# TomBeacock/volumetric-renderer

Hardware: AMD Instinct MI355X
Metric: Gsamples/sec + fps, 512³ NRRD @ 1080p; achieved HBM GB/s vs peak (higher is better)
Workload: dtype f32

## Files before the change

include/vr/vr.h:

```cpp
#ifndef VR_VR_H
#define VR_VR_H

#include <stddef.h>
#include <stdint.h>

#ifdef __cplusplus
extern "C" {
#endif

#define VR_ABI_VERSION 9

#define VR_OK 0
#define VR_EINVAL (-22)
#define VR_ENOMEM (-12)
#define VR_ENODEV (-19)
#define VR_ENODATA (-61)
#define VR_EIO (-5)

enum vr_dtype {
    VR_DTYPE_I8 = 1,
    VR_DTYPE_U8 = 2,
    VR_DTYPE_I16 = 3,
    VR_DTYPE_U16 = 4,
    VR_DTYPE_I32 = 5,
// ... 32 lines not shown
    int32_t wave_shape;
    int32_t frames_in_flight;
    int32_t exact_gradient;
    int32_t depth_zero_to_one;
} vr_params;

typedef struct vr_stats {
    uint64_t rays;
    uint64_t samples;
    uint64_t shaded_samples;
    uint64_t steps;
    uint64_t skipped_samples;
} vr_stats;

int vr_abi_version(void);
void vr_params_default(vr_params *p);

typedef struct vr_ctx vr_ctx;
vr_ctx *vr_create(int device, uint32_t width, uint32_t height);
vr_ctx *vr_create_mask(uint32_t device_mask, uint32_t width, uint32_t height);
void vr_destroy(vr_ctx *ctx);
const char *vr_last_error(const vr_ctx *ctx);

int vr_resize(vr_ctx *ctx, uint32_t width, uint32_t height);
int vr_get_size(const vr_ctx *ctx, uint32_t *width, uint32_t *height);
int vr_get_device(const vr_ctx *ctx, int *device);
int vr_get_device_mask(const vr_ctx *ctx, uint32_t *device_mask);


int vr_set_volume(vr_ctx *ctx, const void *data, int dtype, uint32_t nx, uint32_t ny,
                  uint32_t nz, float vmin, float vmax);
int vr_set_volume_device(vr_ctx *ctx, const void *data_dev, int dtype, uint32_t nx,
                         uint32_t ny, uint32_t nz, float vmin, float vmax, void *stream);
int vr_generate_volume(vr_ctx *ctx, int kind, int dtype, uint32_t nx, uint32_t ny,
                       uint32_t nz, uint32_t seed, float *vmin_out, float *vmax_out);
uint64_t vr_volume_bytes(const vr_ctx *ctx);
int vr_debug_read_volume(vr_ctx *ctx, float *out_host);
int vr_debug_read_volume_native(vr_ctx *ctx, void *out_host);
int vr_debug_volume_info(const vr_ctx *ctx, uint32_t dims[3], float minmax[2], int *storage);

int vr_set_transfer_function(vr_ctx *ctx, const uint32_t *rgba8_srgb, uint32_t n);

int vr_set_slicing(vr_ctx *ctx, const float min_slice[3], const float max_slice[3]);


int vr_render(vr_ctx *ctx, const vr_camera *cam, const vr_params *p, void *out,
              int out_format);

int vr_render_device(vr_ctx *ctx, const vr_camera *cam, const vr_params *p, void *out_dev,
                     int out_format, uint32_t row_block, uint32_t rank, uint32_t nranks,
                     void *stream);
uint32_t vr_shard_rows(uint32_t height, uint32_t row_block, uint32_t nranks);
int vr_set_row_share(vr_ctx *ctx, uint32_t first_weight, uint32_t other_weight);
int vr_get_row_share(const vr_ctx *ctx, uint32_t *first_weight, uint32_t *other_weight);
uint32_t vr_shard_rows_ctx(const vr_ctx *ctx, uint32_t height, uint32_t row_block, uint32_t nranks);
int vr_assemble_rows(vr_ctx *ctx, const void *gathered_dev, void *out_dev, int out_format,
                     uint32_t row_block, uint32_t nranks, void *stream);

typedef struct vr_external_memory vr_external_memory;
int vr_import_memory_fd(vr_ctx *ctx, int fd, uint64_t size, uint64_t offset,
                        vr_external_memory **mem, void **dev_ptr);
int vr_release_external_memory(vr_ctx *ctx, vr_external_memory *mem);

typedef struct vr_memory_info {
    uint64_t volume_bytes;
    uint64_t field_bytes;
    uint64_t oblique_copy_bytes;
    uint64_t plain_copy_bytes;
    uint64_t stencil_copy_bytes;
    uint64_t skip_bytes;
    uint64_t derived_bytes;
    uint64_t budget_bytes;
    uint64_t builds;
    uint64_t evictions;
    uint64_t downgrades;
    uint64_t last_downgrade;
} vr_memory_info;
enum vr_derived {
    VR_DERIVED_FIELD = 1,
    VR_DERIVED_OBLIQUE_COPY = 2,
    VR_DERIVED_PLAIN_COPY = 3,
    VR_DERIVED_STENCIL_COPY = 4,
    VR_DERIVED_SKIP = 5,
    VR_DERIVED_YMAJOR_COPY = 6
};
#define VR_MEMORY_BUDGET_UNLIMITED (~(uint64_t)0)
#define VR_MEMORY_BUDGET_DEFAULT (~(uint64_t)0 - 1)
int vr_set_memory_budget(vr_ctx *ctx, uint64_t bytes);
int vr_memory_report(const vr_ctx *ctx, vr_memory_info *out);
int vr_prepare(vr_ctx *ctx, const vr_camera *cam, const vr_params *p);

int vr_count_work(vr_ctx *ctx, const vr_camera *cam, const vr_params *p, uint32_t row_block,
                  uint32_t rank, uint32_t nranks, vr_stats *out);

int vr_timing_enable(vr_ctx *ctx, int enable);
int vr_timing_read(vr_ctx *ctx, double *total_ms, uint64_t *launches);
int vr_timing_reset(vr_ctx *ctx);

const char *vr_kernel_name(const vr_ctx *ctx, const vr_params *p);

#ifdef __cplusplus
}
#endif

#endif
```

include/vr/vr_debug.h:

```cpp
#ifndef VR_VR_DEBUG_H
#define VR_VR_DEBUG_H

#include "vr.h"
#include "vr_dist.h"

#ifdef __cplusplus
extern "C" {
#endif

enum vr_knob {
    VR_KNOB_PIPELINE = 1,
    VR_KNOB_PAIR = 2,
    VR_KNOB_PAIR_LANES = 3,
    VR_KNOB_GRAD_FIELD = 4,
    VR_KNOB_U8_LAYOUT = 6,
    VR_KNOB_TILE_ORDER = 7,
    VR_KNOB_NARROW = 8,
    VR_KNOB_ALT_GEOMETRY = 9,
    VR_KNOB_MIP_INFLIGHT = 10
};

typedef struct vr_member_timing {
    int32_t device;
    uint64_t frames;
    double kernel_ms, render_ms, gather_ms, assemble_ms;
} vr_member_timing;
int vr_debug_timing_member(vr_ctx *ctx, int member, vr_member_timing *out);

enum vr_exchange { VR_EXCHANGE_RCCL = 0, VR_EXCHANGE_COPY = 1 };
vr_ctx *vr_debug_create_members(const int *devices, int n, uint32_t width, uint32_t height,
                                int exchange);
int vr_debug_fail_member(vr_ctx *ctx, int member, uint64_t frame);

int vr_debug_host_profile_enable(vr_ctx *ctx, int enable);
int vr_debug_host_profile_member(vr_ctx *ctx, int member, vr_dist_host_profile *out);

int vr_debug_set_knob(vr_ctx *ctx, int knob, int value);
int vr_debug_get_knob(const vr_ctx *ctx, int knob, int *value);

typedef struct vr_variant_facts {
    int32_t layout, mode;
    int32_t shade, count, skip, field, field_half, pipeline;
    int32_t tf_n, pair, mip_inflight;
} vr_variant_facts;
int vr_debug_variant_name(const vr_variant_facts *facts, char *buf, size_t n);
const char *vr_debug_last_kernel_name(const vr_ctx *ctx);

uint64_t vr_debug_ymajor_copy_bytes(const vr_ctx *ctx);

#ifdef __cplusplus
}
#endif

#endif
```

volumetric-renderer_amd/csrc/vr_api.hip:

```cpp
#include "../../include/vr/vr.h"
#include "../../include/vr/vr_debug.h"
#include "../../include/vr/vr_modes.h"
#include "../../include/vr/vr_iso.h"
#include "../../include/vr/vr_mpr.h"
#include "vr_internal.h"
#include "vr_group.h"

#include <algorithm>
#include <cmath>
#include <cstdio>
#include <cstdlib>
#include <cstring>
#include <new>
#include <string>
#include <vector>

#pragma clang fp contract(off)

using namespace vr;

#ifndef VR_HOST_BANDS
#define VR_HOST_BANDS 4
#endif
constexpr int kRenderBands = VR_HOST_BANDS;

struct vr_ctx {
    int device = 0;
    uint32_t width = 0, height = 0;
    void *bricks = nullptr;
    size_t brick_bytes = 0;
    int storage = ST_F32;
    int layout = ST_F32;
    bool dense_rows = false;
    double pixel_span = 0.0;
    double axis_align = 1.0;
    int ray_axis = 2;
    double row_align = 1.0;
    struct AltCopy {
        void *bricks = nullptr;
        size_t bytes = 0;
        bool valid = false, failed = false;
        uint64_t used = 0;
    } alt[4];
    uint32_t nx = 1, ny = 1, nz = 1;
    float vmin = 0.0f, vmax = 1.0f;
    float4 *tf = nullptr;
    uint32_t tf_n = 0;
    uint32_t *tf_nz = nullptr;
    float smin[3] = {0.0f, 0.0f, 0.0f};
    float smax[3] = {1.0f, 1.0f, 1.0f};
    int render_mode = VR_MODE_COMPOSITE;
    float isovalue = 0.0f;
    float2 *brick_range = nullptr;
    uint8_t *skip_dist = nullptr;
    size_t nbricks_alloc = 0;
    bool range_valid = false, dist_valid = false;
    float *grad = nullptr;
    size_t grad_bytes = 0;
    bool grad_valid = false;
    uint64_t grad_used = 0;
    bool grad_half = false;
    int grad_scale_log2 = 0;
    float data_lo = 0.0f, data_hi = 1.0f;
    struct TileSched {
        uint32_t tiles_x = 0, tiles_y = 0, supers_x = 0, per_xcd = 0;
        uint32_t row_block = 0, rank = 0, nranks = 0, share_w0 = 1, share_w = 1;
        int pair = 0;
        uint32_t kernel = 0;
        void *stream = nullptr;
        uint32_t *cost = nullptr, *perm = nullptr, *lists = nullptr;
        bool have_perm = false;
        uint32_t launches = 0;
    };
    std::vector<TileSched> sched;
    hipEvent_t built_ev = nullptr;
    bool built_recorded = false;
    struct Fence {
        hipStream_t stream;
        hipEvent_t ev;
        uint64_t used;
        bool external;
        uint64_t build_seen;
    };
    std::vector<Fence> fences;
    uint64_t build_gen = 0;
    uint64_t frame_no = 0;
    FrameVariant last_variant;
    std::string last_mpr_name;
    uint64_t n_builds = 0, n_evictions = 0, n_downgrades = 0;
    uint32_t last_downgrade = 0;
    unsigned long long *counters = nullptr;
    void *frame_dev = nullptr;
    size_t frame_bytes = 0;
    void *mpr_dev = nullptr;
    size_t mpr_bytes = 0;
    hipStream_t band_stream[2] = {nullptr, nullptr};
    hipStream_t copy_stream = nullptr;
    hipEvent_t band_ev[kRenderBands] = {};
    bool timing = false;
    std::vector<hipEvent_t> ev_pool;
    std::vector<std::pair<hipEvent_t, hipEvent_t>> ev_pending;
    double timed_ms = 0.0;
    uint64_t timed_launches = 0;
    struct Knobs {
        int pipeline = -1, pair = -1, pair_lanes = 0, grad_field = -1, u8_layout = -1,
            tile_order = 0, narrow = 1, alt = -1, mip_inflight = 0;
    } knobs;
    std::vector<vr_ctx *> members;
    vr::Group *group = nullptr;
    uint32_t device_mask = 0;
    hipStream_t group_stream = nullptr;
    RowShare share{1, 1};
    uint64_t budget = VR_MEMORY_BUDGET_DEFAULT;
    std::string err;
};

namespace {

thread_local std::string g_err;

int fail(vr_ctx *c, int code, const std::string &msg)
{
    if (c)
        c->err = msg;
    else
        g_err = msg;
    return code;
}

int hip_fail(vr_ctx *c, hipError_t e, const char *what)
{
    std::string m = std::string(what) + ": " + hipGetErrorString(e);
    (void)hipGetLastError();
    return fail(c, e == hipErrorOutOfMemory ? VR_ENOMEM : VR_EIO, m);
}

#define HIP_TRY(c, expr, what)                        \
    do {                                              \
        hipError_t _e = (expr);                       \
        if (_e != hipSuccess) return hip_fail(c, _e, what); \
    } while (0)

int wait_idle(vr_ctx *c)
{
    HIP_TRY(c, hipSetDevice(c->device), "hipSetDevice");
    HIP_TRY(c, hipDeviceSynchronize(), "hipDeviceSynchronize (resource swap)");
    return VR_OK;
}

int storage_for(int dtype)
{
    switch (dtype) {
        case VR_DTYPE_U8: return ST_U8;
        case VR_DTYPE_I8: return ST_I8;
        case VR_DTYPE_U16: return ST_U16;
        case VR_DTYPE_I16: return ST_I16;
        case VR_DTYPE_I32:
        case VR_DTYPE_U32:
        case VR_DTYPE_I64:
        case VR_DTYPE_U64:
        case VR_DTYPE_F32:
        case VR_DTYPE_F64: return ST_F32;
        default: return -1;
    }
}

size_t dtype_size(int dtype)
{
    switch (dtype) {
        case VR_DTYPE_U8:
        case VR_DTYPE_I8: return 1;
        case VR_DTYPE_U16:
        case VR_DTYPE_I16: return 2;
        case VR_DTYPE_I32:
        case VR_DTYPE_U32:
        case VR_DTYPE_F32: return 4;
        default: return 8;
    }
}

void glm_mul(const float *a, const float *b, float *r)
{
    float t[16];
    for (int j = 0; j < 4; ++j)
        for (int i = 0; i < 4; ++i) {
            float acc = a[0 * 4 + i] * b[j * 4 + 0];
            acc = acc + a[1 * 4 + i] * b[j * 4 + 1];
            acc = acc + a[2 * 4 + i] * b[j * 4 + 2];
            acc = acc + a[3 * 4 + i] * b[j * 4 + 3];
// ... 85 lines not shown
    a[15] = m[0] * m[5] * m[10] - m[0] * m[6] * m[9] - m[4] * m[1] * m[10] +
            m[4] * m[2] * m[9] + m[8] * m[1] * m[6] - m[8] * m[2] * m[5];
    const double det = m[0] * a[0] + m[1] * a[4] + m[2] * a[8] + m[3] * a[12];
    if (det == 0.0) return false;
    const double id = 1.0 / det;
    for (int i = 0; i < 16; ++i) inv[i] = a[i] * id;
    return true;
}

bool unprojection(const vr_camera *cam, uint32_t W, uint32_t H, bool zo, double *inv)
{
    const float fovy = (cam->fovy_deg > 0.0f ? cam->fovy_deg : 40.0f) *
                       0.01745329251994329576923690768489f;
    const float zn = cam->znear > 0.0f ? cam->znear : 0.1f;
    const float zf = cam->zfar > 0.0f ? cam->zfar : 10.0f;
    const float aspect = (float)W / (float)H;
    float persp[16], conv[16], proj[16], pv[16];
    if (zo)
        perspective_rh_zo(fovy, aspect, zn, zf, persp);
    else
        perspective_rh_no(fovy, aspect, zn, zf, persp);
    coordinate_conversion(conv);
    glm_mul(persp, conv, proj);
    glm_mul(proj, cam->view, pv);
    double pvd[16];
    for (int i = 0; i < 16; ++i) pvd[i] = (double)pv[i];
    return inverse4d(pvd, inv);
}

float srgb_to_linear(uint32_t c8)
{
    const double c = (double)c8 / 255.0;
    const double l = c <= 0.04045 ? c / 12.92 : std::pow((c + 0.055) / 1.055, 2.4);
    return (float)l;
}

struct SplitMix {
    uint64_t s;
    uint64_t next()
    {
        uint64_t z = (s += 0x9E3779B97F4A7C15ull);
        z = (z ^ (z >> 30)) * 0xBF58476D1CE4E5B9ull;
        z = (z ^ (z >> 27)) * 0x94D049BB133111EBull;
        return z ^ (z >> 31);
    }
    float uniform() { return (float)(next() >> 40) * (1.0f / 16777216.0f); }
};

int brick_layout(const vr_ctx *c, int st, uint32_t nx, uint32_t ny, uint32_t nz)
{
    if (!VR_U8_PLAIN || (st != ST_U8 && st != ST_I8)) return st;
    bool quad = (size_t)nx * ny * nz <= kQuadMaxVoxels;
    if (c->knobs.u8_layout >= 0) quad = c->knobs.u8_layout == 1;
    return quad ? (st | kQuadFlag) : st;
}

int narrow_storage(vr_ctx *c, const void *data_dev, int dtype, size_t count, hipStream_t s,
                   int *st)
{
    int *r = reinterpret_cast<int *>(c->counters);
    const int init[3] = {0x7FFFFFFF, (int)0x80000000, 0};
    HIP_TRY(c, hipMemcpyAsync(r, init, sizeof init, hipMemcpyHostToDevice, s), "hipMemcpy(range)");
    HIP_TRY(c, launch_int_range(dtype, data_dev, count, r, s), "integer range kernel");
    int h[3];
    HIP_TRY(c, hipMemcpyAsync(h, r, sizeof h, hipMemcpyDeviceToHost, s), "hipMemcpy(range)");
    HIP_TRY(c, hipStreamSynchronize(s), "integer range sync");
    if (h[2]) return VR_OK;
    if (h[0] >= 0 && h[1] <= 255)
        *st = ST_U8;
    else if (h[0] >= -128 && h[1] <= 127)
        *st = ST_I8;
    else if (h[0] >= 0 && h[1] <= 65535)
        *st = ST_U16;
    else if (h[0] >= -32768 && h[1] <= 32767)
        *st = ST_I16;
    return VR_OK;
}

void free_derived(vr_ctx *c);

int set_bricks(vr_ctx *c, int storage, uint32_t nx, uint32_t ny, uint32_t nz, void **out)
{
    c->range_valid = c->dist_valid = false;
    c->grad_valid = false;
    for (auto &a : c->alt) a.valid = a.failed = false;
    const size_t bytes = (size_t)bricks_for(nx, 0, storage) * bricks_for(ny, 1, storage) *
                         bricks_for(nz, 2, storage) * brick_elems(storage) * element_size(storage);
    if (c->bricks && c->brick_bytes == bytes) {
        *out = c->bricks;
        return VR_OK;
    }
    free_derived(c);
    if (c->bricks) {
        hipFree(c->bricks);
        c->bricks = nullptr;
        c->brick_bytes = 0;
    }
    void *p = nullptr;
    hipError_t e = hipMalloc(&p, bytes + kBrickSlackBytes);
    if (e != hipSuccess) return hip_fail(c, e, "hipMalloc(volume bricks)");
    c->bricks = p;
    c->brick_bytes = bytes;
    *out = p;
    return VR_OK;
}

int data_range(vr_ctx *c, hipStream_t s)
{
    c->data_lo = 0.0f;
    c->data_hi = 0.0f;
    if (c->storage != ST_F32) return VR_OK;
    uint32_t *mm = reinterpret_cast<uint32_t *>(c->counters);
    const uint32_t init[2] = {0xFFFFFFFFu, 0u};
    HIP_TRY(c, hipMemcpyAsync(mm, init, sizeof init, hipMemcpyHostToDevice, s), "hipMemcpy(range)");
    HIP_TRY(c, launch_minmax(ST_F32, c->bricks, c->brick_bytes / sizeof(float),
                             reinterpret_cast<float *>(mm), s),
            "data range kernel");
    uint32_t h[2];
    HIP_TRY(c, hipMemcpyAsync(h, mm, sizeof h, hipMemcpyDeviceToHost, s), "hipMemcpy(range)");
    HIP_TRY(c, hipStreamSynchronize(s), "data range sync");
    auto unorder = [](uint32_t o) {
        const uint32_t u = (o & 0x80000000u) ? (o & 0x7FFFFFFFu) : ~o;
        float f;
        std::memcpy(&f, &u, 4);
        return f;
    };
    c->data_lo = unorder(h[0]);
    c->data_hi = unorder(h[1]);
    return VR_OK;
}

int upload_tf(vr_ctx *c, const uint32_t *tf, uint32_t n)
{
    std::vector<float4> col(n);
    for (uint32_t i = 0; i < n; ++i) {
        const uint32_t t = tf[i];
        col[i] = make_float4(srgb_to_linear(t & 0xFFu), srgb_to_linear((t >> 8) & 0xFFu),
                             srgb_to_linear((t >> 16) & 0xFFu), (float)((t >> 24) & 0xFFu) / 255.0f);
    }
    std::vector<float4> lut(2 * ((size_t)n + 2), make_float4(0.0f, 0.0f, 0.0f, 0.0f));
    for (uint32_t i = 0; i < n; ++i) {
        const float4 a = col[i], b = i + 1 < n ? col[i + 1] : a;
        lut[2 * (i + 1)] = a;
        lut[2 * (i + 1) + 1] = make_float4(b.x - a.x, b.y - a.y, b.z - a.z, b.w - a.w);
    }
    lut[0] = col[0];
    lut[2 * ((size_t)n + 1)] = col[n - 1];
    if (c->tf && c->tf_n != n) {
        hipFree(c->tf);
        hipFree(c->tf_nz);
        c->tf = nullptr;
        c->tf_nz = nullptr;
    }
    std::vector<uint32_t> nz(n + 1);
    nz[0] = 0;
    for (uint32_t i = 0; i < n; ++i) nz[i + 1] = nz[i] + ((tf[i] >> 24) != 0u ? 1u : 0u);
    if (!c->tf) {
        HIP_TRY(c, hipMalloc(&c->tf, 2 * ((size_t)n + 2) * sizeof(float4)), "hipMalloc(TF)");
        HIP_TRY(c, hipMalloc(&c->tf_nz, (n + 1) * sizeof(uint32_t)), "hipMalloc(TF alpha prefix)");
    }
    HIP_TRY(c, hipMemcpy(c->tf, lut.data(), lut.size() * sizeof(float4), hipMemcpyHostToDevice),
            "hipMemcpy(TF)");
    HIP_TRY(c, hipMemcpy(c->tf_nz, nz.data(), (n + 1) * sizeof(uint32_t), hipMemcpyHostToDevice),
            "hipMemcpy(TF alpha prefix)");
    c->tf_n = n;
    c->dist_valid = false;
    return VR_OK;
// ... 42 lines not shown
        d[a] = f[a] - o[a];
        od += o[a] * d[a];
        dd += d[a] * d[a];
    }
    if (!(dd > 0.0)) return false;
    *align = std::fmax(std::fabs(d[0]), std::fmax(std::fabs(d[1]), std::fabs(d[2]))) / std::sqrt(dd);
    *axis = std::fabs(d[0]) >= std::fabs(d[1]) ? (std::fabs(d[0]) >= std::fabs(d[2]) ? 0 : 2)
                                               : (std::fabs(d[1]) >= std::fabs(d[2]) ? 1 : 2);
    const double t = -od / dd;
    double n2 = 0.0, v2 = 0.0;
    const double nv[3] = {(double)nx, (double)ny, (double)nz};
    for (int a = 0; a < 3; ++a) {
        s[a] = (o2[a] + t * (f2[a] - o2[a])) - (o[a] + t * d[a]);
        n2 += s[a] * s[a];
        v2 += (s[a] * nv[a]) * (s[a] * nv[a]);
    }
    if (!(n2 > 0.0)) return false;
    *span = std::sqrt(v2);
    *row_align = std::fabs(s[0]) / std::sqrt(n2);
    return *row_align >= 0.9 && *span <= 0.8;
}

constexpr double kAltAlign = 0.9, kAltSpan = 0.8, kRowsAlign = 0.97;
bool use_grad_field(const vr_ctx *c, bool half)
{
    if (c->storage != ST_F32) return false;
    if (c->knobs.grad_field >= 0) return c->knobs.grad_field == 1;
    if (c->dense_rows) return true;
    if (!half || c->axis_align < kAltAlign || c->ray_axis == 0) return false;
    return c->pixel_span <= kAltSpan || (c->ray_axis == 2 && c->row_align >= kRowsAlign);
}

bool use_pipeline(bool shading, uint32_t tiles, const vr_ctx *c)
{
    if (c->knobs.pipeline >= 0) return c->knobs.pipeline == 1;
    const size_t voxels = (size_t)c->nx * c->ny * c->nz;
    return tiles * (kThreadsPerTile / 64) < kPipelineMaxWaves ||
           c->brick_bytes >= kPipelineMinBytes || voxels >= kPipelineMinVoxels || c->dense_rows ||
           (shading && c->storage == ST_F32);
}

int want_alt(const vr_ctx *c, const vr_params *p, bool pair, bool field, bool field_half,
             bool pipelined);
bool use_pair(const vr_ctx *c, const MarchParams &P, const vr_params *p)
{
    if (p->skip_empty || P.tf_n > kTfLds) return false;
    if (c->knobs.pair >= 0) return c->knobs.pair == 1;
    if (p->frames_in_flight >= 2) return false;
    if (!p->shading) return false;
    if (P.tiles_x * P.tiles_y * (kThreadsPerTile / 64) < kPairMaxWaves) return true;
    if (c->knobs.alt >= 0 || c->layout != ST_F32 || c->dense_rows || c->pixel_span <= kAltSpan ||
        (c->ray_axis == 2 && c->axis_align >= kAltAlign))
        return false;
    return want_alt(c, p, P.pair != 0, P.grad != nullptr, P.grad_half != 0, P.pipelined != 0) ==
           (ST_F32 | kAltFlag);
}

int build_params(vr_ctx *c, const vr_camera *cam, const vr_params *p, void *out,
                 int out_format, uint32_t row_block, uint32_t rank, uint32_t nranks,
                 RowShare share, MarchParams &P)
{
    if (!cam) return fail(c, VR_EINVAL, "camera is NULL");
    int rc = check_params(c, p);
    if (rc) return rc;
    if (out_format != VR_OUT_RGBA8 && out_format != VR_OUT_RGBA32F)
        return fail(c, VR_EINVAL, "unknown out_format");
    if (nranks == 0 || rank >= nranks || row_block == 0)
        return fail(c, VR_EINVAL, "bad shard (row_block, rank, nranks)");
    std::memset(&P, 0, sizeof(P));
    if (!unprojection(cam, c->width, c->height, p->depth_zero_to_one != 0, P.inv))
        return fail(c, VR_EINVAL, "proj * view is singular");
    P.vol = c->bricks;
    P.vol_bytes = c->brick_bytes;
    P.tf = c->tf;
    P.out = out;
    P.counters = c->counters;
    P.fw = (double)c->width;
    P.fh = (double)c->height;
    P.nx = c->nx;
    P.ny = c->ny;
    P.nz = c->nz;
    P.nbx = bricks_for(c->nx, 0, c->layout);
    P.nby = bricks_for(c->ny, 1, c->layout);
    P.fnx = (float)c->nx;
    P.fny = (float)c->ny;
    P.fnz = (float)c->nz;
    P.vmin = c->vmin;
    P.range = c->vmax - c->vmin;
    P.div_fast = P.range >= 0x1p-40f && P.range < 0x1p100f && std::fabs(c->vmin) < 0x1p100f &&
                 std::fabs(c->vmax) < 0x1p100f;
    P.inv_range = P.div_fast ? 1.0f / P.range : 0.0f;
    P.tf_n = (int32_t)c->tf_n;
    P.tf_nf = (float)c->tf_n;
    for (int a = 0; a < 3; ++a) {
        P.smin[a] = c->smin[a];
        P.smax[a] = c->smax[a];
        P.cam[a] = cam->position[a];
    }
    P.step = p->step;
    P.nsteps = (int32_t)(p->ray_dist / p->step);
    P.ert_eps = p->ert_eps;
    for (int k = 0; k < 4; ++k) P.clear[k] = p->clear_color[k];
    P.ka = p->ambient;
    P.kd = p->diffuse;
    P.ks = p->specular;
    P.spec_power = p->spec_power;
    P.W = c->width;
    P.H = c->height;
    P.row_block = row_block;
    P.rank = rank;
    P.nranks = nranks;
    P.local_rows = share_shard_rows(c->height, row_block, nranks, share);
    P.out_bytes = (unsigned long long)P.local_rows * c->width * (out_format == VR_OUT_RGBA32F ? 16 : 4);
    P.share_w0 = share.w0;
    P.share_w = share.w;
    P.tiles_x = (c->width + 15) / 16;
    P.tiles_y = (P.local_rows + kMarchRows - 1) / kMarchRows;
    P.tile_order = p->tile_order >= 1 && p->tile_order <= 4 ? (uint32_t)p->tile_order : 4u;
    if (p->tile_order == 0 && c->knobs.tile_order >= 1)
        P.tile_order = (uint32_t)c->knobs.tile_order;
    P.wave_w_shift = p->wave_shape == 1 ? 3u : (p->wave_shape == 3 ? 2u : 4u);
    while ((64u >> P.wave_w_shift) > kMarchRows) ++P.wave_w_shift;
    P.supers_x = (P.tiles_x + kSuper - 1) / kSuper;
    P.supers_total = P.supers_x * ((P.tiles_y + kSuper - 1) / kSuper);
    P.out_format = out_format;
    P.slab_default = c->smin[0] == 0.0f && c->smin[1] == 0.0f && c->smin[2] == 0.0f &&
                     c->smax[0] == 1.0f && c->smax[1] == 1.0f && c->smax[2] == 1.0f;
    c->dense_rows = view_dense_rows(P.inv, c->width, c->nx, c->ny, c->nz, &c->pixel_span,
                                    &c->axis_align, &c->ray_axis, &c->row_align);
    P.pipelined = use_pipeline(p->shading != 0, P.tiles_x * P.tiles_y, c);
    return VR_OK;
}

vr_ctx::Fence *fence_of(vr_ctx *c, hipStream_t s)
{
    for (auto &x : c->fences)
        if (x.stream == s) return &x;
    return nullptr;
}
int record_build(vr_ctx *c, hipStream_t s)
{
    if (!c->built_ev)
        HIP_TRY(c, hipEventCreateWithFlags(&c->built_ev, hipEventDisableTiming), "hipEventCreate");
    HIP_TRY(c, hipEventRecord(c->built_ev, s), "hipEventRecord(build)");
    c->built_recorded = true;
    ++c->build_gen;
    if (vr_ctx::Fence *f = fence_of(c, s)) f->build_seen = c->build_gen;
    return VR_OK;
}

constexpr size_t kSkipBytesPerBrick = sizeof(float2) + 2;
size_t derived_bytes(const vr_ctx *c)
{
    size_t b = c->grad ? c->grad_bytes : 0;
    for (const auto &a : c->alt)
        if (a.bricks) b += a.bytes + kBrickSlackBytes;
    return b + c->nbricks_alloc * kSkipBytesPerBrick;
}
constexpr uint64_t kDerivedBudgetBricks = 5;
uint64_t effective_budget(const vr_ctx *c)
{
    if (c->budget != VR_MEMORY_BUDGET_DEFAULT) return c->budget;
    return kDerivedBudgetBricks * (uint64_t)c->brick_bytes + (uint64_t)c->brick_bytes / 32 +
           64ull * kBrickSlackBytes;
}
bool budget_allows(const vr_ctx *c, size_t extra, size_t replaced)
{
    if (c->budget == VR_MEMORY_BUDGET_UNLIMITED) return true;
    const size_t now = derived_bytes(c) - replaced;
    return now + extra <= effective_budget(c);
}
constexpr size_t kMaxFences = 32;
#ifndef VR_FENCE_SYSTEM_SCOPE
#define VR_FENCE_SYSTEM_SCOPE 0
#endif
constexpr unsigned kFenceEventFlags =
    hipEventDisableTiming | (VR_FENCE_SYSTEM_SCOPE ? 0u : (unsigned)hipEventDisableSystemFence);
int fence_record(vr_ctx *c, hipStream_t s)
{
    vr_ctx::Fence *f = fence_of(c, s);
    if (f && f->external) {
        f->used = c->frame_no;
        return VR_OK;
    }
    if (!f) {
        if (c->fences.size() < kMaxFences) {
            hipEvent_t e = nullptr;
            HIP_TRY(c, hipEventCreateWithFlags(&e, kFenceEventFlags), "hipEventCreate(fence)");
            c->fences.push_back(vr_ctx::Fence{s, e, 0, false, 0});
            f = &c->fences.back();
        } else {
            vr_ctx::Fence *old = nullptr;
            for (auto &x : c->fences)
                if (!x.external && (!old || x.used < old->used)) old = &x;
            if (!old) return VR_OK;
            HIP_TRY(c, hipEventSynchronize(old->ev), "hipEventSynchronize(fence)");
            old->stream = s;
            old->build_seen = 0;
            f = old;
        }
    }
    f->used = c->frame_no;
    HIP_TRY(c, hipEventRecord(f->ev, s), "hipEventRecord(fence)");
    return VR_OK;
}
int fence_others(vr_ctx *c, hipStream_t s)
{
    for (const auto &x : c->fences)
        if (x.stream != s && hipStreamWaitEvent(s, x.ev, 0) != hipSuccess) {
            (void)hipGetLastError();
            HIP_TRY(c, hipDeviceSynchronize(), "hipDeviceSynchronize (fence fallback)");
            for (size_t i = c->fences.size(); i-- > 0;)
                if (!c->fences[i].external) {
                    hipEventDestroy(c->fences[i].ev);
                    c->fences.erase(c->fences.begin() + (long)i);
                }
            return VR_OK;
        }
    return VR_OK;
}
int release_async(vr_ctx *c, void *p, hipStream_t s)
{
    if (!p) return VR_OK;
    if (int rc = fence_others(c, s)) return rc;
    HIP_TRY(c, hipFreeAsync(p, s), "hipFreeAsync(derived structure)");
    return VR_OK;
}
constexpr int kYMajorAlt = 3;
int make_room(vr_ctx *c, size_t extra, size_t replaced, int keep_alt, bool keep_field, hipStream_t s,
              bool *fits)
{
    *fits = budget_allows(c, extra, replaced);
    while (!*fits) {
        int pick = -2;
        uint64_t oldest = ~0ull;
        if (c->grad && !keep_field && c->grad_used < oldest) {
            pick = -1;
            oldest = c->grad_used;
        }
        for (int i = 0; i < (int)(sizeof c->alt / sizeof c->alt[0]); ++i)
            if (i != keep_alt && c->alt[i].bricks && c->alt[i].used < oldest) {
                pick = i;
                oldest = c->alt[i].used;
            }
        if (keep_alt != kYMajorAlt && c->alt[kYMajorAlt].bricks) pick = kYMajorAlt;
        if (pick == -2) return VR_OK;
        if (pick == -1) {
            if (int rc = release_async(c, c->grad, s)) return rc;
            c->grad = nullptr;
            c->grad_bytes = 0;
            c->grad_valid = false;
        } else {
            if (int rc = release_async(c, c->alt[pick].bricks, s)) return rc;
            c->alt[pick] = vr_ctx::AltCopy();
        }
        ++c->n_evictions;
        *fits = budget_allows(c, extra, replaced);
    }
    return VR_OK;
}
void free_derived(vr_ctx *c)
{
    if (c->grad) (void)hipFreeAsync(c->grad, nullptr);
    c->grad = nullptr;
    c->grad_bytes = 0;
    c->grad_valid = false;
    for (auto &a : c->alt) {
        if (a.bricks) (void)hipFreeAsync(a.bricks, nullptr);
        a = vr_ctx::AltCopy();
    }
    if (c->brick_range) hipFree(c->brick_range);
    if (c->skip_dist) hipFree(c->skip_dist);
    c->brick_range = nullptr;
    c->skip_dist = nullptr;
    c->nbricks_alloc = 0;
    c->range_valid = c->dist_valid = false;
    (void)hipStreamSynchronize(nullptr);
}

int alloc_skip(vr_ctx *c, size_t nb, bool *have)
{
    *have = false;
    if (nb > 0xFFFFFFFFull) return fail(c, VR_EINVAL, "skip_empty: too many bricks");
    if (c->nbricks_alloc != nb && !budget_allows(c, nb * kSkipBytesPerBrick, c->nbricks_alloc * kSkipBytesPerBrick))
        return VR_OK;
    if (c->nbricks_alloc != nb) {
        if (c->brick_range) hipFree(c->brick_range);
        if (c->skip_dist) hipFree(c->skip_dist);
        c->brick_range = nullptr;
        c->skip_dist = nullptr;
        c->nbricks_alloc = 0;
        c->range_valid = c->dist_valid = false;
        HIP_TRY(c, hipMalloc(&c->brick_range, (nb + 1) * sizeof(float2)), "hipMalloc(brick ranges)");
        HIP_TRY(c, hipMalloc(&c->skip_dist, 2 * nb), "hipMalloc(skip distance field)");
        c->nbricks_alloc = nb;
    }
    *have = true;
    return VR_OK;
}
int build_ranges(vr_ctx *c, size_t nb, hipStream_t s)
{
    if (c->range_valid) return VR_OK;
    HIP_TRY(c, launch_brick_range(c->layout, c->bricks, bricks_for(c->nx, 0, c->layout), bricks_for(c->ny, 1, c->layout),
                                  bricks_for(c->nz, 2, c->layout), c->brick_range, s),
            "brick range kernel");
    HIP_TRY(c, launch_range_max(c->brick_range, (uint32_t)nb, s), "brick range maximum kernel");
    c->range_valid = true;
    c->dist_valid = false;
    return VR_OK;
}
size_t brick_count(const vr_ctx *c)
{
    return (size_t)bricks_for(c->nx, 0, c->layout) * bricks_for(c->ny, 1, c->layout) * bricks_for(c->nz, 2, c->layout);
}

int ensure_skip(vr_ctx *c, MarchParams &P, hipStream_t s)
{
    const size_t nb = brick_count(c);
    bool have = false;
    if (int rc = alloc_skip(c, nb, &have)) return rc;
    if (!have) return VR_OK;
    if (!c->range_valid || !c->dist_valid) ++c->n_builds;
    if (int rc = build_ranges(c, nb, s)) return rc;
    if (!c->dist_valid) {
        HIP_TRY(c, launch_skip_dist(c->brick_range, bricks_for(c->nx, 0, c->layout), bricks_for(c->ny, 1, c->layout),
                                    bricks_for(c->nz, 2, c->layout), c->tf_nz, (int)c->tf_n, c->vmin,
                                    c->vmax - c->vmin, c->skip_dist, c->skip_dist + nb, s),
                "skip distance kernels");
        c->dist_valid = true;
    }
    P.skip_dist = c->skip_dist;
    P.skip_empty = 1;
    return VR_OK;
}

int ensure_mip_ranges(vr_ctx *c, MarchParams &P, MipArgs &M, hipStream_t s)
{
    const size_t nb = brick_count(c);
    bool have = false;
    if (int rc = alloc_skip(c, nb, &have)) return rc;
    if (!have) return VR_OK;
    if (!c->range_valid) ++c->n_builds;
    if (int rc = build_ranges(c, nb, s)) return rc;
    M.brick_range = c->brick_range;
    M.nbricks = (uint32_t)nb;
    P.skip_empty = 1;
    return VR_OK;
}

bool ensure_grad(vr_ctx *c, MarchParams &P, hipStream_t s, bool half, bool *refused)
{
    bool built = false;
    *refused = false;
    if (!use_grad_field(c, half)) return built;
    *refused = true;
    const int k = half ? field_scale_log2(c->data_lo, c->data_hi) : 0;
    if (c->grad_valid && (c->grad_half != half || c->grad_scale_log2 != k)) {
        if (fence_others(c, s) != VR_OK) {
            (void)hipGetLastError();
            return built;
        }
        c->grad_valid = false;
    }
    const size_t bytes = c->brick_bytes / element_size(ST_F32) * kGradElemBytes;
    if (!c->grad || c->grad_bytes != bytes) {
        if (c->grad && release_async(c, c->grad, s) != VR_OK) return built;
        c->grad = nullptr;
        c->grad_bytes = 0;
        c->grad_valid = false;
        bool fits = false;
        if (make_room(c, bytes, 0, -1, false, s, &fits) != VR_OK || !fits) return built;
        size_t free_b = 0, total_b = 0;
        if (hipMemGetInfo(&free_b, &total_b) != hipSuccess || free_b < bytes + (2ull << 30))
            return built;
        void *g = nullptr;
        if (hipMallocAsync(&g, bytes, s) != hipSuccess) {
            (void)hipGetLastError();
            return built;
        }
        c->grad = static_cast<float *>(g);
        c->grad_bytes = bytes;
    }
    if (!c->grad_valid) {
        if (launch_grad_field(static_cast<const float *>(c->bricks), c->grad, c->nx, c->ny, c->nz,
                              half, k, s) != hipSuccess)
            return built;
        built = true;
        ++c->n_builds;
        c->grad_valid = true;
        c->grad_half = half;
        c->grad_scale_log2 = k;
    }
    *refused = false;
    P.grad = c->grad;
    P.grad_half = half ? 1 : 0;
    c->grad_used = c->frame_no;
    return built;
}

int wait_builds(vr_ctx *c, hipStream_t s)
{
    if (c->built_recorded) {
        vr_ctx::Fence *f = fence_of(c, s);
        if (!f || f->build_seen != c->build_gen) {
            HIP_TRY(c, hipStreamWaitEvent(s, c->built_ev, 0), "hipStreamWaitEvent(build)");
            if (f) f->build_seen = c->build_gen;
        }
    }
    return VR_OK;
}
int ensure_derived(vr_ctx *c, const vr_params *p, MarchParams &P, hipStream_t s, uint32_t *refused)
{
    if (int rc = wait_builds(c, s)) return rc;
    const bool r0 = c->range_valid, d0 = c->dist_valid;
    if (p->skip_empty) {
        int rc = ensure_skip(c, P, s);
        if (rc) return rc;
        if (!P.skip_empty) *refused = VR_DERIVED_SKIP;
    }
    bool g_refused = false;
    const bool g_built = p->shading && ensure_grad(c, P, s, p->exact_gradient == 0, &g_refused);
    if (g_refused) *refused = VR_DERIVED_FIELD;
    const bool built = (!r0 && c->range_valid) || (!d0 && c->dist_valid) || g_built;
    if (built) return record_build(c, s);
    return VR_OK;
}

int ensure_mip(vr_ctx *c, const vr_params *p, MarchParams &P, MipArgs &M, hipStream_t s,
               uint32_t *refused)
{
    if (int rc = wait_builds(c, s)) return rc;
    M.brick_range = nullptr;
    M.nbricks = 0;
    P.pipelined = 0;
    if (!p->skip_empty) return VR_OK;
    const bool r0 = c->range_valid;
    if (int rc = ensure_mip_ranges(c, P, M, s)) return rc;
    if (!P.skip_empty) *refused = VR_DERIVED_SKIP;
    if (!r0 && c->range_valid) return record_build(c, s);
    return VR_OK;
}
int mip_inflight(const vr_ctx *c, bool skip)
{
    if (c->knobs.mip_inflight) return c->knobs.mip_inflight;
    if (c->layout == ST_F32 && c->pixel_span > kAltSpan) return skip ? 4 : 1;
    if ((c->layout & kQuadFlag) && skip) return 4;
    return kMipDefaultInFlight;
}

int iso_inflight(const vr_ctx *c, bool skip)
{
    if (c->knobs.mip_inflight) return c->knobs.mip_inflight;
    if (c->layout == ST_F32 && c->pixel_span > kAltSpan) return skip ? 4 : 1;
    if (c->layout == ST_U16 || c->layout == ST_I16) return mip_inflight(c, skip);
    if (c->layout & kQuadFlag) return 4;
    return skip ? 2 : 4;
}
int proj_inflight(const vr_ctx *c, bool skip)
{
    if (c->knobs.mip_inflight) return c->knobs.mip_inflight;
    if (c->render_mode == VR_MODE_MEAN && c->layout == ST_F32 && !skip && c->pixel_span <= kAltSpan)
        return 4;
    return mip_inflight(c, skip);
}
bool proj_mode(const vr_ctx *c)
{
    return c->render_mode == VR_MODE_MINIP || c->render_mode == VR_MODE_MEAN;
}
int range_inflight(const vr_ctx *c, bool skip)
{
    return c->render_mode == VR_MODE_ISO ? iso_inflight(c, skip)
           : proj_mode(c)                ? proj_inflight(c, skip)
                                         : mip_inflight(c, skip);
}
bool range_mode(const vr_ctx *c)
{
    return c->render_mode == VR_MODE_MIP || c->render_mode == VR_MODE_ISO || proj_mode(c);
}
IsoArgs iso_args(const vr_ctx *c, const vr_params *p, const MipArgs &M)
{
    return {M.brick_range, M.nbricks, c->isovalue, p->shading != 0};
}

constexpr size_t kInfinityCacheBytes = 256ull << 20;
bool knobs_default(const vr_ctx *c)
{
    const vr_ctx::Knobs &k = c->knobs;
    return k.pipeline < 0 && k.pair < 0 && k.pair_lanes == 0 && k.grad_field < 0 && k.alt < 0 &&
           k.tile_order == 0;
}
bool want_ymajor(const vr_ctx *c, const vr_params *p, bool field, bool field_half, bool pipelined)
{
    if (!pipelined || c->tf_n > (uint32_t)kTfLds) return false;
    if (p->shading ? !(field && field_half && p->exact_gradient == 0) : field) return false;
    if (c->knobs.alt >= 0) return c->knobs.alt == 5;
    return knobs_default(c) && c->dense_rows && c->ray_axis == 1 &&
           c->brick_bytes > kInfinityCacheBytes;
}
int want_alt(const vr_ctx *c, const vr_params *p, bool pair, bool field, bool field_half,
             bool pipelined)
{
    if (c->layout != ST_F32 || p->skip_empty || pair) return c->layout;
    if (want_ymajor(c, p, field, field_half, pipelined)) return ST_F32 | kYMajorFlag;
    if (field) return c->layout;
    int which = 0;
    if (c->knobs.alt >= 0)
        which = c->knobs.alt;
    else if (!c->dense_rows) {
        if (c->pixel_span > kAltSpan && c->row_align >= kRowsAlign)
            which = p->shading ? 4 : 3;
        else if (c->axis_align >= kAltAlign && c->ray_axis != 0 && c->pixel_span <= kAltSpan)
            which = 0;
        else
            which = 1;
    }
    switch (which) {
        case 1: return ST_F32 | kAltFlag;
        case 3: return ST_F32 | kPlainF32Flag;
        case 4: return ST_F32 | kStencilF32Flag;
        default: return c->layout;
    }
}

int alt_index(int layout)
{
    if (layout & kAltFlag) return 0;
    if (layout & kYMajorFlag) return kYMajorAlt;
    return (layout & kPlainF32Flag) ? 1 : 2;
}
uint32_t alt_derived_code(int layout)
{
    return (layout & kYMajorFlag) ? (uint32_t)VR_DERIVED_YMAJOR_COPY
                                  : (uint32_t)(VR_DERIVED_OBLIQUE_COPY + alt_index(layout));
}

size_t alt_bytes_for(const vr_ctx *c, int lay)
{
    return (size_t)bricks_for(c->nx, 0, lay) * bricks_for(c->ny, 1, lay) * bricks_for(c->nz, 2, lay) *
           brick_elems(lay) * element_size(lay);
}

int ensure_alt(vr_ctx *c, int lay, hipStream_t s, bool *ready)
{
    *ready = false;
    vr_ctx::AltCopy &a = c->alt[alt_index(lay)];
    const size_t bytes = alt_bytes_for(c, lay);
    if (a.valid && a.bricks && a.bytes == bytes) {
        *ready = true;
        a.used = c->frame_no;
        return VR_OK;
    }
    if (a.failed) return VR_OK;
    if (!a.bricks || a.bytes != bytes) {
        const size_t had = a.bricks ? a.bytes + kBrickSlackBytes : 0;
        bool fits = false;
        if (lay & kYMajorFlag)
            fits = budget_allows(c, bytes + kBrickSlackBytes, had);
        else if (int rc = make_room(c, bytes + kBrickSlackBytes, had, alt_index(lay), false, s, &fits))
            return rc;
        if (!fits) return VR_OK;
        if (int rc = release_async(c, a.bricks, s)) return rc;
        a.bricks = nullptr;
        a.bytes = 0;
        size_t free_b = 0, total_b = 0;
        if (hipMemGetInfo(&free_b, &total_b) != hipSuccess ||
            free_b < bytes + kBrickSlackBytes + (2ull << 30) ||
            hipMallocAsync(&a.bricks, bytes + kBrickSlackBytes, s) != hipSuccess) {
            (void)hipGetLastError();
            a.bricks = nullptr;
            a.failed = true;
            return VR_OK;
        }
        a.bytes = bytes;
    }
    const hipError_t e = launch_rebrick_f32(static_cast<const float *>(c->bricks), a.bricks, c->nx,
                                            c->ny, c->nz, lay, s);
    if (e != hipSuccess) return hip_fail(c, e, "alt geometry copy");
    a.valid = true;
    a.used = c->frame_no;
    ++c->n_builds;
    *ready = true;
    return record_build(c, s);
}

VariantFacts launch_facts(const vr_ctx *c, const vr_params *p, const MarchParams &P, int layout,
                          bool count)
{
    const bool skip = P.skip_empty != 0;
    const int k = range_mode(c) ? range_inflight(c, skip) : 0;
    return {layout, c->render_mode, p->shading != 0, count, skip, P.grad != nullptr, P.grad_half,
            P.pipelined, P.tf_n, P.pair, k};
}
VariantFacts next_frame_facts(const vr_ctx *c, const vr_params *p)
{
    VariantFacts f{};
    f.layout = c->layout;
    f.mode = c->render_mode;
    f.shade = p && p->shading;
    f.tf_n = (int32_t)c->tf_n;
    if (range_mode(c)) {
        f.skip = p && p->skip_empty && c->range_valid && c->nbricks_alloc;
        f.mip_inflight = range_inflight(c, f.skip);
        return f;
    }
    f.skip = p && p->skip_empty;
    f.field = f.shade && use_grad_field(c, p->exact_gradient == 0) && c->grad && c->grad_valid;
    f.field_half = f.field && p->exact_gradient == 0;
    const uint32_t tiles = ((c->width + 15) / 16) * ((c->height + kMarchRows - 1) / kMarchRows);
    f.pipeline = use_pipeline(f.shade, tiles, c);
    if (p)
        if (const int lay = want_alt(c, p, false, f.field != 0, f.field_half != 0, f.pipeline != 0);
            lay != c->layout && c->alt[alt_index(lay)].valid)
            f.layout = lay;
    return f;
}

vr_ctx::TileSched *tile_sched(vr_ctx *c, MarchParams &P, void *stream, uint32_t kernel)
{
    if (P.tile_order != 4) return nullptr;
    auto use = [&P](vr_ctx::TileSched &t) {
        P.tile_cost = t.cost;
        if (t.have_perm) {
            P.tile_perm = t.perm;
            P.nperm = 8 * t.per_xcd;
        }
    };
    for (auto &t : c->sched)
        if (t.tiles_x == P.tiles_x && t.tiles_y == P.tiles_y && t.pair == P.pair &&
            t.kernel == kernel &&
            t.stream == stream && t.row_block == P.row_block && t.rank == P.rank &&
            t.nranks == P.nranks && t.share_w0 == P.share_w0 && t.share_w == P.share_w) {
            use(t);
            return &t;
        }
    if (c->sched.size() >= kMaxTileScheds) {
        hipFree(c->sched.front().cost);
        hipFree(c->sched.front().perm);
        hipFree(c->sched.front().lists);
        c->sched.erase(c->sched.begin());
    }
    vr_ctx::TileSched t;
    t.tiles_x = P.tiles_x;
    t.tiles_y = P.tiles_y;
    t.supers_x = P.supers_x;
    t.pair = P.pair;
    t.kernel = kernel;
    t.stream = stream;
    t.row_block = P.row_block;
    t.rank = P.rank;
    t.nranks = P.nranks;
    t.share_w0 = P.share_w0;
    t.share_w = P.share_w;
    std::vector<std::vector<uint32_t>> xl(8);
    if (VR_LIST_ORDER == 1) {
        const uint32_t sy_n = (P.tiles_y + kSuper - 1) / kSuper;
        for (uint32_t sy = 0; sy < sy_n; ++sy)
            for (uint32_t sx = 0; sx < P.supers_x; ++sx)
                for (uint32_t w = 0; w < kSuper * kSuper; ++w) {
                    const uint32_t tx = sx * kSuper + w % kSuper, ty = sy * kSuper + w / kSuper;
                    if (tx < P.tiles_x && ty < P.tiles_y)
                        xl[(sy * P.supers_x + sx) & 7u].push_back(ty * P.tiles_x + tx);
                }
    } else {
        for (uint32_t ty = 0; ty < P.tiles_y; ++ty)
            for (uint32_t tx = 0; tx < P.tiles_x; ++tx)
                xl[((ty >> kSuperShift) * P.supers_x + (tx >> kSuperShift)) & 7u].push_back(
                    ty * P.tiles_x + tx);
    }
    for (int x = 0; x < 8; ++x) t.per_xcd = xl[x].size() > t.per_xcd ? (uint32_t)xl[x].size() : t.per_xcd;
    std::vector<uint32_t> lists(8 * (size_t)t.per_xcd, 0xFFFFFFFFu);
    for (int x = 0; x < 8; ++x)
        std::copy(xl[x].begin(), xl[x].end(), lists.begin() + (size_t)x * t.per_xcd);
    const size_t nt = (size_t)P.tiles_x * P.tiles_y;
    hipStream_t hs = static_cast<hipStream_t>(stream);
    if (hipMalloc(&t.cost, nt * sizeof(uint32_t)) != hipSuccess ||
        hipMalloc(&t.perm, lists.size() * sizeof(uint32_t)) != hipSuccess ||
        hipMalloc(&t.lists, lists.size() * sizeof(uint32_t)) != hipSuccess ||
        hipMemcpyAsync(t.lists, lists.data(), lists.size() * sizeof(uint32_t),
                       hipMemcpyHostToDevice, hs) != hipSuccess) {
        (void)hipGetLastError();
        hipFree(t.cost);
        hipFree(t.perm);
        hipFree(t.lists);
        return nullptr;
    }
    c->sched.push_back(t);
    use(c->sched.back());
    return &c->sched.back();
}

bool is_group(const vr_ctx *c) { return c && c->group; }

int group_idle(vr_ctx *c)
{
    std::string m;
    if (vr::group_synchronize(c->group, &m) != VR_OK) return fail(c, VR_EIO, m);
    return VR_OK;
}

int replicate_volume(vr_ctx *c)
{
    vr_ctx *src = c->members[0];
    const size_t n = c->members.size();
    std::vector<hipStream_t> st(n, nullptr);
    int rc = VR_OK;
    for (size_t k = 1; k < n && rc == VR_OK; ++k) {
        vr_ctx *d = c->members[k];
        if ((rc = wait_idle(d)) != VR_OK) break;
        void *dst = nullptr;
        if ((rc = set_bricks(d, src->layout, src->nx, src->ny, src->nz, &dst)) != VR_OK) break;
        hipError_t e = hipStreamCreateWithFlags(&st[k], hipStreamNonBlocking);
        if (e == hipSuccess)
            e = hipMemcpyPeerAsync(dst, d->device, src->bricks, src->device, src->brick_bytes, st[k]);
        if (e != hipSuccess) rc = hip_fail(c, e, "replicate volume (peer copy)");
        if (rc == VR_OK) {
            d->storage = src->storage;
            d->layout = src->layout;
            d->nx = src->nx;
            d->ny = src->ny;
            d->nz = src->nz;
            d->vmin = src->vmin;
            d->vmax = src->vmax;
            d->data_lo = src->data_lo;
            d->data_hi = src->data_hi;
            d->range_valid = d->dist_valid = d->grad_valid = false;
        }
    }
    for (size_t k = 1; k < n; ++k)
        if (st[k]) {
            hipSetDevice(c->members[k]->device);
            const hipError_t e = hipStreamSynchronize(st[k]);
            if (e != hipSuccess && rc == VR_OK) rc = hip_fail(c, e, "replicate volume (sync)");
            hipStreamDestroy(st[k]);
        }
    hipSetDevice(c->device);
    return rc;
}

int member_rc(vr_ctx *c, vr_ctx *m, int rc)
{
    if (rc != VR_OK) c->err = m->err;
    return rc;
}

int *knob_slot(vr_ctx *c, int knob)
{
    switch (knob) {
        case VR_KNOB_PIPELINE: return &c->knobs.pipeline;
        case VR_KNOB_PAIR: return &c->knobs.pair;
        case VR_KNOB_PAIR_LANES: return &c->knobs.pair_lanes;
        case VR_KNOB_GRAD_FIELD: return &c->knobs.grad_field;
        case VR_KNOB_U8_LAYOUT: return &c->knobs.u8_layout;
        case VR_KNOB_TILE_ORDER: return &c->knobs.tile_order;
        case VR_KNOB_NARROW: return &c->knobs.narrow;
        case VR_KNOB_ALT_GEOMETRY: return &c->knobs.alt;
        case VR_KNOB_MIP_INFLIGHT: return &c->knobs.mip_inflight;
        default: return nullptr;
    }
}

bool knob_value_ok(int knob, int v)
{
    switch (knob) {
        case VR_KNOB_PAIR_LANES: return v == 0 || v == 2 || v == 4;
        case VR_KNOB_NARROW: return v == 0 || v == 1;
        case VR_KNOB_ALT_GEOMETRY: return v >= -1 && v <= 5 && v != 2;
        case VR_KNOB_TILE_ORDER: return v >= 0 && v <= 4;
        case VR_KNOB_MIP_INFLIGHT: return v == 0 || v == 1 || v == 2 || v == 4;
        default: return v >= -1 && v <= 1;
    }
}

#ifdef VR_EXPERIMENTS
void knobs_from_env(vr_ctx *c)
{
    auto flag = [](const char *name, int &dst) {
        if (const char *e = std::getenv(name)) dst = e[0] == '1' ? 1 : 0;
    };
    flag("VR_PIPELINE", c->knobs.pipeline);
    flag("VR_PAIR", c->knobs.pair);
    if (const char *e = std::getenv("VR_PAIR_LANES")) c->knobs.pair_lanes = e[0] == '4' ? 4 : 2;
    if (std::getenv("VR_NO_GRAD_FIELD")) c->knobs.grad_field = 0;
    if (std::getenv("VR_GRAD_FIELD_ALWAYS")) c->knobs.grad_field = 1;
    if (const char *e = std::getenv("VR_U8_LAYOUT")) c->knobs.u8_layout = e[0] == 'q' ? 1 : 0;
    if (const char *e = std::getenv("VR_TILE_ORDER_DEFAULT"))
        if (e[0] >= '1' && e[0] <= '4') c->knobs.tile_order = e[0] - '0';
}
#endif

hipEvent_t pooled_event(vr_ctx *c)
{
    if (!c->ev_pool.empty()) {
        hipEvent_t e = c->ev_pool.back();
        c->ev_pool.pop_back();
        return e;
    }
    hipEvent_t e = nullptr;
    if (hipEventCreateWithFlags(&e, hipEventDisableSystemFence) != hipSuccess) return nullptr;
    return e;
}

vr_ctx *create_members(const std::vector<int> &devices, uint32_t width, uint32_t height,
                       int exchange)
{
    if (width == 0 || height == 0) {
        fail(nullptr, VR_EINVAL, "framebuffer size must be non-zero");
        return nullptr;
    }
    vr_ctx *c = new (std::nothrow) vr_ctx();
    if (!c) {
        fail(nullptr, VR_ENOMEM, "out of host memory");
        return nullptr;
    }
    c->device = devices[0];
    for (int d : devices)
        if (d < 32) c->device_mask |= 1u << d;
    c->width = width;
    c->height = height;
#ifdef VR_EXPERIMENTS
    knobs_from_env(c);
#endif
    for (int d : devices) {
        vr_ctx *m = vr_create(d, width, height);
        if (!m) {
            const std::string e = g_err;
            vr_destroy(c);
            fail(nullptr, VR_ENODEV, "device " + std::to_string(d) + ": " + e);
            return nullptr;
        }
        m->knobs = c->knobs;
        c->members.push_back(m);
    }
    std::string err;
    c->group = vr::group_create(c->members, exchange, &err);
    if (!c->group) {
        vr_destroy(c);
        fail(nullptr, VR_ENODEV, "multi-device context: " + err);
        return nullptr;
    }
// ... 599 lines not shown
}

int vr_memory_report(const vr_ctx *c, vr_memory_info *out)
{
    if (!c || !out) return fail(nullptr, VR_EINVAL, "NULL argument");
    if (is_group(c)) return vr_memory_report(c->members[0], out);
    std::memset(out, 0, sizeof *out);
    out->volume_bytes = c->brick_bytes;
    out->field_bytes = c->grad ? c->grad_bytes : 0;
    uint64_t *copies[3] = {&out->oblique_copy_bytes, &out->plain_copy_bytes, &out->stencil_copy_bytes};
    for (int i = 0; i < 3; ++i)
        *copies[i] = c->alt[i].bricks ? c->alt[i].bytes + kBrickSlackBytes : 0;
    out->skip_bytes = c->nbricks_alloc * kSkipBytesPerBrick;
    out->derived_bytes = derived_bytes(c);
    out->budget_bytes = c->budget == VR_MEMORY_BUDGET_UNLIMITED ? c->budget : effective_budget(c);
    out->builds = c->n_builds;
    out->evictions = c->n_evictions;
    out->downgrades = c->n_downgrades;
    out->last_downgrade = c->last_downgrade;
    return VR_OK;
}

int vr_prepare(vr_ctx *c, const vr_camera *cam, const vr_params *p)
{
    if (!c) return fail(nullptr, VR_EINVAL, "ctx is NULL");
    if (is_group(c)) {
        if (int rc = group_idle(c)) return rc;
        for (vr_ctx *m : c->members)
            if (int rc = vr_prepare(m, cam, p)) return member_rc(c, m, rc);
        hipSetDevice(c->device);
        return VR_OK;
    }
    HIP_TRY(c, hipSetDevice(c->device), "hipSetDevice");
    if (int rc = render_device_impl(c, cam, p, c->counters, VR_OUT_RGBA8, 16, 0, 1, c->share,
                                    nullptr, false))
        return rc;
    HIP_TRY(c, hipStreamSynchronize(nullptr), "hipStreamSynchronize (prepare)");
    return VR_OK;
}

int vr_render_device(vr_ctx *c, const vr_camera *cam, const vr_params *p, void *out_dev,
                     int out_format, uint32_t row_block, uint32_t rank, uint32_t nranks,
                     void *stream)
{
    if (!c) return fail(nullptr, VR_EINVAL, "ctx is NULL");
    return render_device_impl(c, cam, p, out_dev, out_format, row_block, rank, nranks, c->share,
                              stream);
}

}
namespace {
int render_device_impl(vr_ctx *c, const vr_camera *cam, const vr_params *p, void *out_dev,
                       int out_format, uint32_t row_block, uint32_t rank, uint32_t nranks,
                       RowShare share, void *stream, bool launch)
{
    if (!out_dev) return fail(c, VR_EINVAL, "output buffer is NULL");
    if (is_group(c)) {
        if (rank != 0 || nranks != 1)
            return fail(c, VR_EINVAL, "a multi-device context renders whole frames (rank 0 of 1)");
        if (!cam) return fail(c, VR_EINVAL, "camera is NULL");
        if (int rc = check_params(c, p)) return rc;
        if (out_format != VR_OUT_RGBA8 && out_format != VR_OUT_RGBA32F)
            return fail(c, VR_EINVAL, "unknown out_format");
        std::string m;
        if (int rc = vr::group_render(c->group, cam, p, out_dev, out_format,
                                      static_cast<hipStream_t>(stream), &m))
            return fail(c, rc, m);
        return VR_OK;
    }
    MarchParams P;
    int rc = build_params(c, cam, p, out_dev, out_format, row_block, rank, nranks, share, P);
    if (rc) return rc;
    HIP_TRY(c, hipSetDevice(c->device), "hipSetDevice");
    hipStream_t s = static_cast<hipStream_t>(stream);
    ++c->frame_no;
    uint32_t refused = 0;
    MipArgs M{nullptr, 0};
    int layout = c->layout;
    const bool mip = range_mode(c);
    if (mip) {
        rc = ensure_mip(c, p, P, M, s, &refused);
        if (rc) return rc;
    } else {
        rc = ensure_derived(c, p, P, s, &refused);
        if (rc) return rc;
        if (use_pair(c, P, p)) {
            P.pair = P.tiles_x * P.tiles_y * (kThreadsPerTile / 64) < kPairQuadMaxWaves ? 4 : 2;
            if (c->knobs.pair_lanes == 2 || c->knobs.pair_lanes == 4) P.pair = c->knobs.pair_lanes;
            const uint32_t th = 16 / P.pair;
            P.tiles_y = (P.local_rows + th - 1) / th;
            P.supers_total = P.supers_x * ((P.tiles_y + kSuper - 1) / kSuper);
        }
        if (const int lay = want_alt(c, p, P.pair != 0, P.grad != nullptr, P.grad_half != 0,
                                     P.pipelined != 0);
            lay != c->layout) {
            bool ready = false;
            rc = ensure_alt(c, lay, s, &ready);
            if (rc) return rc;
            if (ready) {
                layout = lay;
                P.vol = c->alt[alt_index(lay)].bricks;
                P.vol_bytes = c->alt[alt_index(lay)].bytes;
                P.nbx = bricks_for(c->nx, 0, layout);
                P.nby = bricks_for(c->ny, 1, layout);
            } else {
                if (!(lay & kYMajorFlag) || c->knobs.alt == 5) refused = alt_derived_code(lay);
            }
        }
    }
    if (!launch) return VR_OK;
    if (refused) {
        ++c->n_downgrades;
        c->last_downgrade = refused;
    }
    FrameVariant v;
    resolve_variant(launch_facts(c, p, P, layout, false), &v);
    vr_ctx::TileSched *ts = tile_sched(c, P, stream, variant_tile_key(v, layout));
    hipEvent_t e0 = nullptr, e1 = nullptr;
    const bool timing = c->timing;
    if (timing) {
        e0 = pooled_event(c);
        e1 = pooled_event(c);
        if (!e0 || !e1) return fail(c, VR_EIO, "hipEventCreate failed");
        HIP_TRY(c, hipEventRecord(e0, s), "hipEventRecord");
    }
    HIP_TRY(c, launch_frame(v, P, M, iso_args(c, p, M), s),
            v.family == VF_ISO    ? "iso kernel launch"
            : v.family == VF_PROJ ? "proj kernel launch"
            : mip                 ? "mip kernel launch"
                                  : "march kernel launch");
    c->last_variant = v;
    c->last_mpr_name.clear();
    if (timing) {
        HIP_TRY(c, hipEventRecord(e1, s), "hipEventRecord");
        c->ev_pending.emplace_back(e0, e1);
    }
    if (ts && ts->launches++ % kReorderEvery == 0) {
        HIP_TRY(c, launch_order_tiles(ts->cost, ts->lists, ts->perm, ts->per_xcd, s),
                "tile order kernel");
        ts->have_perm = true;
    }
    return fence_record(c, s);
}
}
extern "C" {

int vr_render(vr_ctx *c, const vr_camera *cam, const vr_params *p, void *out, int out_format)
{
    if (!c) return fail(nullptr, VR_EINVAL, "ctx is NULL");
    if (!out) return fail(c, VR_EINVAL, "output buffer is NULL");
    if (!p) return fail(c, VR_EINVAL, "params is NULL");
    HIP_TRY(c, hipSetDevice(c->device), "hipSetDevice");
    const size_t bpp = out_format == VR_OUT_RGBA32F ? 16 : 4;
    const uint32_t W = c->width, H = c->height;
    if (is_group(c)) {
        const size_t fb = (size_t)W * H * bpp;
        if (c->frame_bytes < fb) {
            if (c->frame_dev) hipFree(c->frame_dev);
            c->frame_dev = nullptr;
            c->frame_bytes = 0;
            HIP_TRY(c, hipMalloc(&c->frame_dev, fb), "hipMalloc(frame)");
            c->frame_bytes = fb;
        }
        if (!c->group_stream)
            HIP_TRY(c, hipStreamCreateWithFlags(&c->group_stream, hipStreamNonBlocking),
                    "hipStreamCreate");
        int rc = vr_render_device(c, cam, p, c->frame_dev, out_format, vr::kGroupRowBlock, 0, 1,
                                  c->group_stream);
        if (rc) return rc;
        HIP_TRY(c, hipMemcpyAsync(out, c->frame_dev, fb, hipMemcpyDeviceToHost, c->group_stream),
                "hipMemcpyAsync(frame)");
        HIP_TRY(c, hipStreamSynchronize(c->group_stream), "hipStreamSynchronize(frame)");
        return VR_OK;
    }
    const int nb = H >= kHostBandMinRows ? kRenderBands : 1;
    const uint32_t R = nb == 1 ? 16 : ((H + nb - 1) / nb + 15) / 16 * 16;
    const size_t bytes = (size_t)W * (nb == 1 ? H : (size_t)R * nb) * bpp;
    if (c->frame_bytes < bytes) {
        if (c->frame_dev) hipFree(c->frame_dev);
        c->frame_dev = nullptr;
        c->frame_bytes = 0;
        HIP_TRY(c, hipMalloc(&c->frame_dev, bytes), "hipMalloc(frame)");
        c->frame_bytes = bytes;
    }
    if (nb == 1) {
        int rc = render_device_impl(c, cam, p, c->frame_dev, out_format, 16, 0, 1, RowShare{1, 1},
                                    nullptr);
        if (rc) return rc;
        HIP_TRY(c, hipMemcpy(out, c->frame_dev, (size_t)W * H * bpp, hipMemcpyDeviceToHost),
                "hipMemcpy(frame)");
        return VR_OK;
    }
// ... 50 lines not shown
}

struct vr_external_memory {
    hipExternalMemory_t ext;
    void *ptr;
    int device;
};

int vr_import_memory_fd(vr_ctx *c, int fd, uint64_t size, uint64_t offset,
                        vr_external_memory **mem, void **dev_ptr)
{
    if (!c) return fail(nullptr, VR_EINVAL, "ctx is NULL");
    if (!mem || !dev_ptr) return fail(c, VR_EINVAL, "NULL output");
    *mem = nullptr;
    *dev_ptr = nullptr;
    if (fd < 0 || size == 0 || offset > UINT64_MAX - size)
        return fail(c, VR_EINVAL, "bad fd, size or offset");
    const int device = is_group(c) ? c->members[0]->device : c->device;
    HIP_TRY(c, hipSetDevice(device), "hipSetDevice");
    hipExternalMemoryHandleDesc hd;
    std::memset(&hd, 0, sizeof hd);
    hd.type = hipExternalMemoryHandleTypeOpaqueFd;
    hd.handle.fd = fd;
    hd.size = offset + size;
    hipExternalMemory_t ext = nullptr;
    HIP_TRY(c, hipImportExternalMemory(&ext, &hd), "hipImportExternalMemory");
    hipExternalMemoryBufferDesc bd;
    std::memset(&bd, 0, sizeof bd);
    bd.offset = offset;
    bd.size = size;
    void *ptr = nullptr;
    const hipError_t e = hipExternalMemoryGetMappedBuffer(&ptr, ext, &bd);
    if (e != hipSuccess) {
        (void)hipDestroyExternalMemory(ext);
        return hip_fail(c, e, "hipExternalMemoryGetMappedBuffer");
    }
    *mem = new vr_external_memory{ext, ptr, device};
    *dev_ptr = ptr;
    return VR_OK;
}

int vr_release_external_memory(vr_ctx *c, vr_external_memory *m)
{
    if (!c) return fail(nullptr, VR_EINVAL, "ctx is NULL");
    if (!m) return fail(c, VR_EINVAL, "mem is NULL");
    HIP_TRY(c, hipSetDevice(m->device), "hipSetDevice");
    HIP_TRY(c, hipDeviceSynchronize(), "hipDeviceSynchronize");
    const hipError_t e1 = hipFree(m->ptr);
    const hipError_t e2 = hipDestroyExternalMemory(m->ext);
    delete m;
    if (e1 != hipSuccess) return hip_fail(c, e1, "hipFree(external mapping)");
    if (e2 != hipSuccess) return hip_fail(c, e2, "hipDestroyExternalMemory");
    return VR_OK;
}

int vr_count_work(vr_ctx *c, const vr_camera *cam, const vr_params *p, uint32_t row_block,
                  uint32_t rank, uint32_t nranks, vr_stats *out)
{
    if (!c) return fail(nullptr, VR_EINVAL, "ctx is NULL");
    if (!out) return fail(c, VR_EINVAL, "stats is NULL");
    if (is_group(c)) {
        if (int rc = group_idle(c)) return rc;
        return member_rc(c, c->members[0],
                         vr_count_work(c->members[0], cam, p, row_block, rank, nranks, out));
    }
    HIP_TRY(c, hipSetDevice(c->device), "hipSetDevice");
    const size_t bytes = (size_t)c->width *
                         share_shard_rows(c->height, row_block ? row_block : 1, nranks ? nranks : 1,
                                          c->share) * 4;
    if (c->frame_bytes < bytes) {
        if (c->frame_dev) hipFree(c->frame_dev);
        c->frame_dev = nullptr;
        c->frame_bytes = 0;
        HIP_TRY(c, hipMalloc(&c->frame_dev, bytes), "hipMalloc(frame)");
        c->frame_bytes = bytes;
    }
    MarchParams P;
    int rc = build_params(c, cam, p, c->frame_dev, VR_OUT_RGBA8, row_block, rank, nranks,
                          c->share, P);
    if (rc) return rc;
    uint32_t refused = 0;
    MipArgs M{nullptr, 0};
    const bool mip = range_mode(c);
    rc = mip ? ensure_mip(c, p, P, M, nullptr, &refused) : ensure_derived(c, p, P, nullptr, &refused);
    if (rc) return rc;
    HIP_TRY(c, hipMemset(c->counters, 0, 8 * sizeof(unsigned long long)), "hipMemset(counters)");
    FrameVariant v;
    resolve_variant(launch_facts(c, p, P, c->layout, true), &v);
    HIP_TRY(c, launch_frame(v, P, M, iso_args(c, p, M), nullptr),
            v.family == VF_ISO    ? "iso (count) launch"
            : v.family == VF_PROJ ? "proj (count) launch"
            : mip                 ? "mip (count) launch"
                                  : "march (count) launch");
    c->last_variant = v;
    c->last_mpr_name.clear();
    unsigned long long h[5];
    HIP_TRY(c, hipMemcpy(h, c->counters, sizeof(h), hipMemcpyDeviceToHost), "hipMemcpy(counters)");
    out->rays = h[0];
    out->samples = h[1];
    out->shaded_samples = h[2];
    out->steps = h[3];
    out->skipped_samples = h[4];
    return VR_OK;
}

int vr_timing_enable(vr_ctx *c, int enable)
{
    if (!c) return fail(nullptr, VR_EINVAL, "ctx is NULL");
    if (is_group(c)) {
        if (int rc = group_idle(c)) return rc;
        vr::group_timing_enable(c->group, enable != 0);
    }
    for (vr_ctx *m : c->members) vr_timing_enable(m, enable);
    c->timing = enable != 0;
    return VR_OK;
}

int vr_debug_timing_member(vr_ctx *c, int member, vr_member_timing *out)
{
    if (!c || !out) return fail(c, VR_EINVAL, "NULL argument");
    std::memset(out, 0, sizeof *out);
    if (!is_group(c)) {
        if (member != 0) return fail(c, VR_EINVAL, "no such member");
        out->device = c->device;
        return vr_timing_read(c, &out->kernel_ms, &out->frames);
    }
    double ms[3] = {0.0, 0.0, 0.0};
    uint64_t frames = 0;
    std::string m;
    if (int rc = vr::group_timing_member(c->group, member, ms, &frames, &m)) return fail(c, rc, m);
    vr_ctx *mc = c->members[(size_t)member];
    uint64_t launches = 0;
    if (int rc = vr_timing_read(mc, &out->kernel_ms, &launches)) return member_rc(c, mc, rc);
    hipSetDevice(c->device);
    out->device = mc->device;
    out->frames = frames;
    out->render_ms = ms[0];
    out->gather_ms = ms[1];
    out->assemble_ms = ms[2];
    return VR_OK;
}

int vr_debug_host_profile_enable(vr_ctx *c, int enable)
{
    if (!c) return fail(nullptr, VR_EINVAL, "ctx is NULL");
    if (!is_group(c)) return fail(c, VR_EINVAL, "not a multi-device context");
    vr::group_host_profile_enable(c->group, enable != 0);
    return VR_OK;
}

int vr_debug_host_profile_member(vr_ctx *c, int member, vr_dist_host_profile *out)
{
    if (!c || !out) return fail(c, VR_EINVAL, "NULL argument");
    if (!is_group(c)) return fail(c, VR_EINVAL, "not a multi-device context");
    std::string m;
    if (int rc = vr::group_host_profile_member(c->group, member, out, &m)) return fail(c, rc, m);
    return VR_OK;
}

int vr_debug_fail_member(vr_ctx *c, int member, uint64_t frame)
{
    if (!c) return fail(nullptr, VR_EINVAL, "ctx is NULL");
    if (!is_group(c)) return fail(c, VR_EINVAL, "not a multi-device context");
    std::string m;
    if (int rc = vr::group_fail_member(c->group, member, frame, &m)) return fail(c, rc, m);
    return VR_OK;
}

int vr_timing_read(vr_ctx *c, double *total_ms, uint64_t *launches)
{
    if (!c) return fail(nullptr, VR_EINVAL, "ctx is NULL");
    if (is_group(c)) {
        if (int rc = group_idle(c)) return rc;
        double ms = 0.0;
        uint64_t n = 0;
        for (vr_ctx *m : c->members) {
            double a = 0.0;
            uint64_t b = 0;
            if (int rc = vr_timing_read(m, &a, &b)) return member_rc(c, m, rc);
            ms += a;
            n += b;
        }
        hipSetDevice(c->device);
        if (total_ms) *total_ms = ms;
        if (launches) *launches = n;
        return VR_OK;
    }
    HIP_TRY(c, hipSetDevice(c->device), "hipSetDevice");
    for (auto &pr : c->ev_pending) {
        if (hipEventSynchronize(pr.second) != hipSuccess) {
            (void)hipGetLastError();
            HIP_TRY(c, hipDeviceSynchronize(), "hipDeviceSynchronize (timing)");
        }
        float ms = 0.0f;
        HIP_TRY(c, hipEventElapsedTime(&ms, pr.first, pr.second), "hipEventElapsedTime");
        c->timed_ms += ms;
        c->timed_launches++;
        c->ev_pool.push_back(pr.first);
        c->ev_pool.push_back(pr.second);
    }
    c->ev_pending.clear();
    if (total_ms) *total_ms = c->timed_ms;
    if (launches) *launches = c->timed_launches;
    return VR_OK;
}

int vr_timing_reset(vr_ctx *c)
{
    if (is_group(c)) {
        if (int rc = group_idle(c)) return rc;
        std::string m;
        if (int rc = vr::group_timing_reset(c->group, &m)) return fail(c, rc, m);
        for (vr_ctx *m : c->members)
            if (int rc = vr_timing_reset(m)) return member_rc(c, m, rc);
        return VR_OK;
    }
    double ms;
    uint64_t n;
    int rc = vr_timing_read(c, &ms, &n);
    if (rc) return rc;
    c->timed_ms = 0.0;
    c->timed_launches = 0;
    return VR_OK;
}

const char *vr_kernel_name(const vr_ctx *c, const vr_params *p)
{
    if (!c) return "";
    if (is_group(c)) return vr_kernel_name(c->members[0], p);
    thread_local std::string name;
    FrameVariant v;
    resolve_variant(next_frame_facts(c, p), &v);
    name = variant_kernel_name(v);
    return name.c_str();
}

int vr_debug_variant_name(const vr_variant_facts *facts, char *buf, size_t n)
{
    FrameVariant v;
    if (!facts || !buf || n == 0 || !resolve_variant(*facts, &v)) return VR_EINVAL;
    std::snprintf(buf, n, "%s", variant_kernel_name(v).c_str());
    return VR_OK;
}

const char *vr_debug_last_kernel_name(const vr_ctx *c)
{
    if (!c) return "";
    if (is_group(c)) return vr_debug_last_kernel_name(c->members[0]);
    thread_local std::string name;
    name = c->last_mpr_name.empty() ? variant_kernel_name(c->last_variant) : c->last_mpr_name;
    return name.c_str();
}

uint64_t vr_debug_ymajor_copy_bytes(const vr_ctx *c)
{
    if (!c) return 0;
    if (is_group(c)) return vr_debug_ymajor_copy_bytes(c->members[0]);
    const vr_ctx::AltCopy &a = c->alt[kYMajorAlt];
    return a.bricks ? a.bytes + kBrickSlackBytes : 0;
}

int vr_debug_set_knob(vr_ctx *c, int knob, int value)
{
    if (!c) return fail(nullptr, VR_EINVAL, "ctx is NULL");
    int *k = knob_slot(c, knob);
    if (!k) return fail(c, VR_EINVAL, "unknown knob");
    if (!knob_value_ok(knob, value)) return fail(c, VR_EINVAL, "knob value out of range");
    if (is_group(c))
        if (int rc = group_idle(c)) return rc;
    *k = value;
    for (vr_ctx *m : c->members) vr_debug_set_knob(m, knob, value);
    return VR_OK;
}

int vr_debug_get_knob(const vr_ctx *c, int knob, int *value)
{
    if (!c || !value) return fail(nullptr, VR_EINVAL, "NULL argument");
    int *k = knob_slot(const_cast<vr_ctx *>(c), knob);
    if (!k) return fail(nullptr, VR_EINVAL, "unknown knob");
    *value = *k;
    return VR_OK;
}

}

namespace {
int check_plane_shape(vr_ctx *c, uint32_t width, uint32_t height, uint32_t nsamples, int op)
{
    if (width == 0 || height == 0) return fail(c, VR_EINVAL, "mpr image size must be non-zero");
    if ((unsigned long long)((width + 15ull) / 16) * ((height + 15ull) / 16) >= 1ull << 31)
        return fail(c, VR_EINVAL, "mpr image too large");
    if (nsamples == 0 || nsamples > VR_MPR_MAX_SAMPLES)
        return fail(c, VR_EINVAL, "mpr nsamples must be in [1, 4096]");
    if (op != VR_MPR_MAX && op != VR_MPR_MIN && op != VR_MPR_MEAN)
        return fail(c, VR_EINVAL, "unknown mpr op");
    return VR_OK;
}

int build_mpr(vr_ctx *c, const vr_mpr_plane *pl, const vr_params *p, void *out, int out_format,
              MprArgs &A)
{
    if (!pl) return fail(c, VR_EINVAL, "plane is NULL");
    if (int rc = check_params(c, p)) return rc;
    for (int a = 0; a < 3; ++a)
        if (!std::isfinite(pl->origin[a]) || !std::isfinite(pl->du[a]) || !std::isfinite(pl->dv[a]) ||
            !std::isfinite(pl->dn[a]))
            return fail(c, VR_EINVAL, "mpr plane vectors must be finite");
    if (int rc = check_plane_shape(c, pl->width, pl->height, pl->nsamples, pl->op)) return rc;
    if (out_format != VR_OUT_RGBA8 && out_format != VR_OUT_RGBA32F)
        return fail(c, VR_EINVAL, "unknown out_format");
    std::memset(&A, 0, sizeof(A));
    A.vol = c->bricks;
    A.vol_bytes = c->brick_bytes;
    A.tf = c->tf;
    A.out = out;
    A.counters = c->counters;
    for (int a = 0; a < 3; ++a) {
        A.origin[a] = (double)pl->origin[a];
        A.du[a] = (double)pl->du[a];
        A.dv[a] = (double)pl->dv[a];
        A.dn[a] = (double)pl->dn[a];
        A.smin[a] = c->smin[a];
        A.smax[a] = c->smax[a];
    }
    A.half_w = 0.5 * (double)pl->width;
    A.half_h = 0.5 * (double)pl->height;
    A.half_n = 0.5 * (double)(pl->nsamples - 1);
    A.nbx = bricks_for(c->nx, 0, c->layout);
    A.nby = bricks_for(c->ny, 1, c->layout);
    A.fnx = (float)c->nx;
    A.fny = (float)c->ny;
    A.fnz = (float)c->nz;
    A.vmin = c->vmin;
    A.range = c->vmax - c->vmin;
// ... 149 lines not shown
```

volumetric-renderer_amd/csrc/vr_internal.h:

```cpp
#pragma once

#include <hip/hip_runtime.h>
#include <stddef.h>
#include <stdint.h>

#include <cmath>
#include <type_traits>

#include "vr_variant.h"

namespace vr {

#ifndef VR_BRICK_CELLS
#define VR_BRICK_CELLS 8, 8, 8
#endif
#ifndef VR_BRICK_ALIGN
#define VR_BRICK_ALIGN 1
#endif
template <int X, int Y, int Z, int LO = 0>
struct BrickGeom {
    static constexpr int BX = X, BY = Y, BZ = Z;
    static constexpr int Lo = LO;
    static constexpr int EX = X + 1 + 2 * LO, EY = Y + 1 + 2 * LO, EZ = Z + 1 + 2 * LO;
    static constexpr int Row = EX, Slice = EX * EY;
// ... 34 lines not shown
                                                                  uint32_t nby)
{
    if constexpr (kGroupShift == 0) {
        return (bz * nby + by) * nbx + bx;
    } else {
        constexpr uint32_t G = kGroupShift;
        const uint32_t grp = ((bz >> G) * (nby >> G) + (by >> G)) * (nbx >> G) + (bx >> G);
        return (grp << (3 * G)) | morton_spread(bx & kGroupMask) |
               (morton_spread(by & kGroupMask) << 1) | (morton_spread(bz & kGroupMask) << 2);
    }
}

__host__ __device__ __forceinline__ void brick_coords(uint32_t slot, uint32_t nbx, uint32_t nby,
                                                      uint32_t &bx, uint32_t &by, uint32_t &bz)
{
    if constexpr (kGroupShift == 0) {
        bx = slot % nbx;
        by = (slot / nbx) % nby;
        bz = slot / (nbx * nby);
    } else {
        constexpr uint32_t G = kGroupShift;
        const uint32_t grp = slot >> (3 * G), m = slot & ((1u << (3 * G)) - 1);
        const uint32_t gx = nbx >> G, gy = nby >> G;
        uint32_t lx = 0, ly = 0, lz = 0;
#pragma unroll
        for (int t = 0; t < (int)G; ++t) {
            lx |= ((m >> (3 * t)) & 1u) << t;
            ly |= ((m >> (3 * t + 1)) & 1u) << t;
            lz |= ((m >> (3 * t + 2)) & 1u) << t;
        }
        bx = ((grp % gx) << G) | lx;
        by = (((grp / gx) % gy) << G) | ly;
        bz = ((grp / (gx * gy)) << G) | lz;
    }
}

constexpr size_t kQuadMaxVoxels = 1ull << 25;
template <typename T>
struct Quad8 {
    T v;
};
#ifndef VR_ALT_BRICK_CELLS
#define VR_ALT_BRICK_CELLS 7, 15, 8
#endif
using GeomAlt = BrickGeom<VR_ALT_BRICK_CELLS>;
struct F32Alt {
    float v;
};
#ifndef VR_PLAIN_BRICK_CELLS
#define VR_PLAIN_BRICK_CELLS 15, 15, 15
#endif
using GeomPlainRows = BrickGeom<VR_PLAIN_BRICK_CELLS>;
struct F32P {
    float v;
};
#ifndef VR_STENCIL_BRICK_CELLS
#define VR_STENCIL_BRICK_CELLS 29, 29, 29
#endif
using GeomStencil = BrickGeom<VR_STENCIL_BRICK_CELLS, 1>;
struct F32S {
    float v;
};
struct F32H {
    float v;
};
struct F32Y {
    float v;
};
struct F32HY {
    float v;
};
__host__ __device__ constexpr uint32_t zmajor_local(uint32_t xl, uint32_t yl, uint32_t zl)
{
    return xl + (uint32_t)GeomWide::EX * (yl + (uint32_t)GeomWide::EY * zl);
}
__host__ __device__ constexpr uint32_t ymajor_local(uint32_t xl, uint32_t yl, uint32_t zl)
{
    return xl + (uint32_t)GeomWide::EX * (zl + (uint32_t)GeomWide::EZ * yl);
}
__host__ __device__ constexpr int ymajor_field_delta(uint32_t yl, uint32_t zl)
{
    return GeomWide::EX * (GeomWide::BY * (int)zl - GeomWide::BZ * (int)yl);
}
__host__ __device__ constexpr size_t ymajor_cell_offset(uint32_t pi, uint32_t pj, uint32_t pk,
                                                        uint32_t nbx, uint32_t nby,
                                                        int *field_delta = nullptr)
{
    using G = GeomWide;
    const uint32_t bx = pi / G::BX, by = pj / G::BY, bz = pk / G::BZ;
    const uint32_t xl = pi - bx * G::BX, yl = pj - by * G::BY, zl = pk - bz * G::BZ;
    if (field_delta) *field_delta = ymajor_field_delta(yl, zl);
    return (size_t)brick_slot(bx, by, bz, nbx, nby) * (size_t)G::Elems + ymajor_local(xl, yl, zl);
}
namespace ymajor_check {
constexpr bool map_ok()
{
    using G = GeomWide;
    constexpr uint32_t nbx = (3 + kGroupMask) & ~kGroupMask, nby = (2 + kGroupMask) & ~kGroupMask,
                       nbz = nby;
    for (uint32_t bz = 0; bz < nbz; ++bz)
        for (uint32_t by = 0; by < nby; ++by)
            for (uint32_t bx = 0; bx < nbx; ++bx) {
                bool seen[G::EX * G::EY * G::EZ] = {};
                const size_t base = (size_t)brick_slot(bx, by, bz, nbx, nby) * (size_t)G::Elems;
                for (uint32_t zl = 0; zl < (uint32_t)G::EZ; ++zl)
                    for (uint32_t yl = 0; yl < (uint32_t)G::EY; ++yl)
                        for (uint32_t xl = 0; xl < (uint32_t)G::EX; ++xl) {
                            const uint32_t l = ymajor_local(xl, yl, zl);
                            if (l >= (uint32_t)(G::EX * G::EY * G::EZ) || seen[l]) return false;
                            seen[l] = true;
                            if ((int)zmajor_local(xl, yl, zl) - (int)l != ymajor_field_delta(yl, zl))
                                return false;
                            if (xl < (uint32_t)G::BX && yl < (uint32_t)G::BY && zl < (uint32_t)G::BZ) {
                                int fd = 0;
                                const size_t e = ymajor_cell_offset(bx * G::BX + xl, by * G::BY + yl,
                                                                    bz * G::BZ + zl, nbx, nby, &fd);
                                if (e != base + l || fd != ymajor_field_delta(yl, zl)) return false;
                            }
                        }
            }
    return true;
}
static_assert(map_ok(), "the y-major map is a bijection onto each brick, 72 (zl - yl) from z-major");
static_assert(GeomWide::BX != 8 || GeomWide::BY != 8 || GeomWide::BZ != 8 ||
                  ymajor_field_delta(3, 5) == 72 * (5 - 3),
              "8^3 cells: l_zmajor - l_ymajor == 72 (zl - yl)");
}

inline size_t storage_size(int st)
{
    switch (st & 0xF) {
        case ST_U8:
        case ST_I8: return 1;
        case ST_U16:
        case ST_I16: return 2;
        default: return 4;
    }
}
inline bool byte_storage(int st)
{
    return VR_U8_PLAIN && !(st & kQuadFlag) && (st == ST_U8 || st == ST_I8);
}
inline size_t voxels_per_element(int st)
{
    if (st & (kPlainF32Flag | kStencilF32Flag)) return 1;
    return (st & 0xF) == ST_F32 ? kF32VoxelsPerElement : (byte_storage(st) ? 1 : 4);
}
inline size_t element_size(int st) { return storage_size(st) * voxels_per_element(st); }
inline int brick_cells(int st, int a)
{
    if (st & kAltFlag) return GeomAlt::cells(a);
    if (st & kPlainF32Flag) return GeomPlainRows::cells(a);
    if (st & kStencilF32Flag) return GeomStencil::cells(a);
    return byte_storage(st) ? GeomByte::cells(a) : GeomWide::cells(a);
}
inline size_t brick_elems(int st)
{
    if (st & kAltFlag) return GeomAlt::Elems;
    if (st & kPlainF32Flag) return GeomPlainRows::Elems;
    if (st & kStencilF32Flag) return GeomStencil::Elems;
    return byte_storage(st) ? GeomByte::Elems : GeomWide::Elems;
}

inline uint32_t bricks_for(uint32_t n, int a, int st)
{
    return ((n + 3) / (uint32_t)brick_cells(st, a) + 1 + kGroupMask) & ~kGroupMask;
}

struct RowShare {
    uint32_t w0, w;
};
__host__ __device__ inline uint32_t share_period(uint32_t n, RowShare s) { return s.w0 + (n - 1) * s.w; }
__host__ __device__ inline uint32_t share_offset(uint32_t r, RowShare s)
{
    return r == 0 ? 0u : s.w0 + (r - 1) * s.w;
}
__host__ __device__ inline uint32_t share_global_block(uint32_t lb, uint32_t r, uint32_t n, RowShare s)
{
    const uint32_t w = r == 0 ? s.w0 : s.w;
    return (lb / w) * share_period(n, s) + share_offset(r, s) + lb % w;
}
__host__ __device__ inline void share_owner(uint32_t gb, uint32_t n, RowShare s, uint32_t &r,
                                            uint32_t &lb)
{
    const uint32_t P = share_period(n, s), q = gb / P, o = gb - q * P;
    if (o < s.w0) {
        r = 0;
        lb = q * s.w0 + o;
    } else {
        const uint32_t t = o - s.w0;
        r = 1 + t / s.w;
        lb = q * s.w + t % s.w;
    }
}
inline uint32_t share_blocks(uint32_t nb, uint32_t r, uint32_t n, RowShare s)
{
    const uint32_t P = share_period(n, s), q = nb / P, o = nb - q * P;
    const uint32_t w = r == 0 ? s.w0 : s.w, off = share_offset(r, s);
    const uint32_t tail = o > off ? (o - off < w ? o - off : w) : 0u;
    return q * w + tail;
}
inline uint32_t share_shard_rows(uint32_t height, uint32_t row_block, uint32_t n, RowShare s)
{
    if (row_block == 0 || n == 0 || s.w0 == 0 || s.w == 0) return 0;
    const uint32_t nb = (height + row_block - 1) / row_block;
    uint32_t m = share_blocks(nb, 0, n, s);
    if (n > 1) {
        const uint32_t b1 = share_blocks(nb, 1, n, s);
        m = b1 > m ? b1 : m;
    }
    return m * row_block;
}

struct MarchParams {
    const void *vol;
    const float4 *tf;
    void *out;
    unsigned long long *counters;

    double inv[16];
    double fw, fh;

    uint32_t nx, ny, nz;
    uint32_t nbx, nby;
    float fnx, fny, fnz;
    float vmin, range;
    int32_t tf_n;
    float tf_nf;

    float smin[3], smax[3];
    float cam[3];
    float step;
    int32_t nsteps;
    float ert_eps;
    float clear[4];
    float ka, kd, ks;
    int32_t spec_power;

    uint32_t W, H;
    uint32_t row_block, rank, nranks, local_rows;
    uint32_t tiles_x, tiles_y;
    uint32_t tile_order;
    uint32_t supers_x, supers_total;
    uint32_t wave_w_shift;
    int32_t out_format;
    int32_t slab_default;
    int32_t pipelined;
    int32_t pair;
    const uint32_t *tile_perm;
    uint32_t *tile_cost;
    uint32_t nperm;
    const uint8_t *skip_dist;
    int32_t skip_empty;
    int32_t div_fast;
    const float *grad;
    int32_t grad_half;
    float inv_range;
    uint32_t share_w0, share_w;
    unsigned long long vol_bytes, out_bytes;
};

struct MipArgs {
    const float2 *brick_range;
    uint32_t nbricks;
};
struct IsoArgs {
    const float2 *brick_range;
    uint32_t nbricks;
    float iso;
    int32_t shading;
};
struct ProjArgs {
    const float2 *brick_range;
    uint32_t nbricks;
};
hipError_t launch_frame(const FrameVariant &v, const MarchParams &p, const MipArgs &m,
                        const IsoArgs &i, hipStream_t stream);
struct MprArgs {
    const void *vol;
    const float4 *tf;
    void *out;
    unsigned long long *counters;
    double origin[3], du[3], dv[3], dn[3];
    double half_w, half_h, half_n;
    uint32_t nbx, nby;
    float fnx, fny, fnz;
    float vmin, range, inv_range;
    int32_t div_fast;
    int32_t tf_n;
    float tf_nf;
    float smin[3], smax[3];
    float clear[4];
    uint32_t W, H, nsamples;
    uint32_t tiles_x, tiles_y;
    uint32_t tile_order, supers_x, supers_total;
    int32_t out_format;
    int32_t op;
    unsigned long long vol_bytes, out_bytes;
};
constexpr int kMprMax = 0, kMprMin = 1, kMprMean = 2, kMprThin = 3;
constexpr uint32_t kMprTileOrder(uint32_t nsamples) { return nsamples == 1 ? 1u : 3u; }
hipError_t launch_mpr(int layout, bool count, const MprArgs &a, hipStream_t stream,
                      std::string *name);
constexpr int kMipDefaultInFlight = 2;
hipError_t launch_range_max(float2 *range_dev, uint32_t nbricks, hipStream_t stream);
constexpr uint32_t kPipelineMaxWaves = 24576;
constexpr size_t kPipelineMinBytes = 4ull << 30;
constexpr size_t kPipelineMinVoxels = 1ull << 29;
#ifndef VR_MARCH_ROWS
#define VR_MARCH_ROWS 16
#endif
constexpr uint32_t kMarchRows = VR_MARCH_ROWS;
#ifndef VR_SUPER_SHIFT
#define VR_SUPER_SHIFT 2
#endif
#ifndef VR_LIST_ORDER
#define VR_LIST_ORDER 0
#endif
constexpr uint32_t kSuperShift = VR_SUPER_SHIFT;
constexpr uint32_t kSuper = 1u << kSuperShift;
constexpr uint32_t kThreadsPerTile = 16 * kMarchRows;
constexpr int kHostBands = 4;
constexpr uint32_t kHostBandMinRows = 256;
hipError_t launch_order_tiles(const uint32_t *cost, const uint32_t *lists, uint32_t *perm,
                              uint32_t per_xcd, hipStream_t stream);
#ifndef VR_REORDER_EVERY
#define VR_REORDER_EVERY 4
#endif
constexpr uint32_t kReorderEvery = VR_REORDER_EVERY;
constexpr size_t kMaxTileScheds = 64;
constexpr uint32_t kPairMaxWaves = 24576;
constexpr uint32_t kPairQuadMaxWaves = 6144;
hipError_t launch_brick_from_linear(int src_dtype, const void *src, void *dst, uint32_t nx,
                                    uint32_t ny, uint32_t nz, int storage, hipStream_t stream);
hipError_t launch_unbrick(int storage, const void *bricks, void *dst, uint32_t nx, uint32_t ny,
                          uint32_t z0, uint32_t cz, hipStream_t stream);
hipError_t launch_generate(int kind, int storage, void *dst_linear, uint32_t nx, uint32_t ny,
                           uint32_t nz, const float *params_dev, int nparams,
                           hipStream_t stream);
hipError_t launch_assemble(const void *gathered, void *out, int out_format, uint32_t W,
                           uint32_t H, uint32_t row_block, uint32_t nranks,
                           uint32_t shard_rows, RowShare share, hipStream_t stream);
hipError_t launch_int_range(int src_dtype, const void *src, size_t count, int *out3_dev,
                            hipStream_t stream);
hipError_t launch_minmax(int storage, const void *linear, size_t count, float *minmax_dev,
                         hipStream_t stream);

constexpr int kSkipCap = 16;
constexpr size_t kGradElemBytes = 24;
hipError_t launch_grad_field(const float *bricks, float *grad, uint32_t nx, uint32_t ny,
                             uint32_t nz, bool half, int scale_log2, hipStream_t stream);
hipError_t launch_rebrick_f32(const float *src_bricks, void *dst, uint32_t nx, uint32_t ny,
                              uint32_t nz, int storage, hipStream_t stream);
inline int field_scale_log2(float vmin, float vmax)
{
    const double B = (double)(vmax > 0.0f ? vmax : 0.0f) - (double)(vmin < 0.0f ? vmin : 0.0f);
    if (!(B > 0.0) || B > 1e300) return 0;
    int k = 0;
    while (k > -120 && B * std::ldexp(1.0, k) > 65504.0) --k;
    while (k < 120 && B * std::ldexp(1.0, k + 1) <= 65504.0) ++k;
    return k;
}
hipError_t launch_brick_range(int storage, const void *bricks, uint32_t nbx, uint32_t nby,
                              uint32_t nbz, float2 *range_dev, hipStream_t stream);
hipError_t launch_skip_dist(const float2 *range_dev, uint32_t nbx, uint32_t nby, uint32_t nbz,
                            const uint32_t *tf_nz_dev, int tf_n, float vmin, float vrange,
                            uint8_t *dist_dev, uint8_t *scratch_dev, hipStream_t stream);

#ifdef VR_WG_TIMES
hipError_t debug_wg_times_reset();
hipError_t debug_wg_times_read(unsigned long long *out, unsigned int max, unsigned int *count);
#endif

}
```

volumetric-renderer_amd/csrc/vr_kernels.hip:

```cpp
#include "vr_exact_math.h"
#include "vr_internal.h"

#include <array>
#include <cstdlib>
#include <tuple>
#include <type_traits>
#include <utility>

#pragma clang fp contract(off)

namespace vr {
namespace {

constexpr int kTile = 16;
constexpr int kThreads = 256;
constexpr int kTfLut = 2 * (kTfLds + 2);

__device__ __forceinline__ float lerpf(float a, float b, float w) { return fmaf(w, b - a, a); }

#ifdef VR_BOUNDS_CHECK
__device__ unsigned int g_oob_reports;
__device__ __noinline__ void oob_report(int what, unsigned long long a, unsigned long long b)
{
    if (atomicAdd(&g_oob_reports, 1u) < 32u)
// ... 950 lines not shown
    if (lane == 0) {
        atomicAdd(&P.counters[0], rays);
        atomicAdd(&P.counters[1], sm);
        atomicAdd(&P.counters[2], sh);
        atomicAdd(&P.counters[3], st);
        atomicAdd(&P.counters[4], sk);
    }
}

template <typename PT>
__device__ __forceinline__ float4 blend_over_clear(const PT &P, float cr, float cg,
                                                   float cb, float T)
{
    const float A = 1.0f - T;
    const float omA = 1.0f - A;
    return make_float4(cr * A + P.clear[0] * omA, cg * A + P.clear[1] * omA,
                       cb * A + P.clear[2] * omA, A * A + P.clear[3] * omA);
}

template <typename PT>
__device__ __forceinline__ void store_pixel(const PT &P, uint32_t px, uint32_t ly,
                                            float4 o)
{
    const size_t idx = (size_t)ly * P.W + px;
    if (VR_OOB(4, idx * (P.out_format == 0 ? 4 : 16), P.out_bytes)) return;
    if (P.out_format == 0) {
        static_cast<uint32_t *>(P.out)[idx] =
            unorm8(o.x) | (unorm8(o.y) << 8) | (unorm8(o.z) << 16) | (unorm8(o.w) << 24);
    } else {
        static_cast<float4 *>(P.out)[idx] = o;
    }
}

__device__ __forceinline__ void stage_tf(const MarchParams &P, float4 *s_tf, int threads)
{
    for (int i = threadIdx.x; i < 2 * (P.tf_n + 2); i += threads) s_tf[i] = P.tf[i];
}

__device__ __forceinline__ void write_tile_cost(const MarchParams &P, uint32_t tile_x,
                                                uint32_t tile_y, long long wg_start)
{
    if (P.tile_cost) {
        __syncthreads();
        if (threadIdx.x == 0)
            P.tile_cost[tile_y * P.tiles_x + tile_x] =
                (uint32_t)min(wall_clock64() - wg_start, 0x7FFFFFFFLL);
    }
}

template <typename VT, bool SHADE, bool COUNT, bool SKIP, bool GF, bool PIPE>
__device__ __forceinline__ void march_strip(const MarchParams &P, LdsF4 *s_tf,
                                            bool tf_in_lds, uint32_t tile_x, uint32_t tile_y,
                                            uint32_t wave, uint32_t lane)
{
    using G = GeomOf<VT>;
    const long by_stride = (long)P.nbx * G::Elems;
    const long bz_stride = (long)P.nbx * P.nby * G::Elems;

    const LanePixel pix = strip_pixel(P, tile_x, tile_y, wave, lane);

    float tex[3] = {0.f, 0.f, 0.f}, dir[3] = {0.f, 0.f, 0.f};
    const bool covered = pix.active && pixel_ray(P, pix.px, pix.gy, tex, dir);

    float T = 1.0f, cr = 0.0f, cg = 0.0f, cb = 0.0f;
    unsigned long long n_samples = 0, n_shaded = 0, n_steps = 0, n_skipped = 0;
    uint32_t cur_brick = 0xFFFFFFFFu, cur_dist = 0;
    const char *__restrict__ vol = static_cast<const char *>(P.vol);
    const int nsteps = covered ? P.nsteps : 0;
    float p0 = tex[0], p1 = tex[1], p2 = tex[2];
    const float d0 = dir[0], d1 = dir[1], d2 = dir[2];
    const int kin = (covered && P.slab_default) ? interior_steps(tex, dir, P.step, nsteps) : 0;
    float inv_du[3] = {0.f, 0.f, 0.f}, leap_margin[3] = {0.f, 0.f, 0.f};
    if (!COUNT && SKIP) {
        const float dd[3] = {d0, d1, d2}, fn[3] = {P.fnx, P.fny, P.fnz};
#pragma unroll
        for (int a = 0; a < 3; ++a) {
            inv_du[a] = 1.0f / (fabsf(dd[a]) * P.step * fn[a]);
            leap_margin[a] = 0.5f + (float)kMaxLeap * 1.2e-7f * fn[a];
        }
    }
    if constexpr (PIPE) {
        struct Stage {
            CellRaw<VT> w;
            size_t ce;
            float ax, ay, az;
            int pi, pj, pk;
            bool ok, slab;
        };
        auto prep = [&](Stage &S, int k, bool live = true) {
            const bool interior = (unsigned)(k - 1) < (unsigned)kin;
            S.ok = live && k < nsteps &&
                   (interior || !(p0 > 1.0f || p1 > 1.0f || p2 > 1.0f || p0 < 0.0f ||
                                  p1 < 0.0f || p2 < 0.0f));
            S.slab = S.ok && (interior || (p0 < P.smax[0] && p1 < P.smax[1] && p2 < P.smax[2] &&
                                           p0 > P.smin[0] && p1 > P.smin[1] && p2 > P.smin[2]));
            int i, j, kk;
            texel_coord(p0, P.fnx, i, S.ax);
            texel_coord(p1, P.fny, j, S.ay);
            texel_coord(p2, P.fnz, kk, S.az);
            if (!S.slab) i = j = kk = 0;
            S.pi = i + kPad;
            S.pj = j + kPad;
            S.pk = kk + kPad;
            if constexpr (kYMajor<VT>) {
                S.ce = cell_offset<float>(S.pi, S.pj, S.pk, P.nbx, P.nby);
                size_t e = (size_t)((long)S.ce -
                                    ymajor_field_delta((uint32_t)S.pj % (uint32_t)G::BY,
                                                       (uint32_t)S.pk % (uint32_t)G::BZ));
                if (VR_OOB(3, e * kElemBytes<VT>, P.vol_bytes)) e = S.ce = 0;
                Cell8<VT>::issue(S.w, vol, e);
            } else {
                S.ce = cell_offset<VT>(S.pi, S.pj, S.pk, P.nbx, P.nby);
                if (VR_OOB(3, S.ce * kElemBytes<VT>, P.vol_bytes)) S.ce = 0;
                Cell8<VT>::issue(S.w, vol, S.ce);
            }
        };
        auto composite = [&](const float4 &sm) -> bool {
            cr = cr + (sm.x * sm.w) * T;
            cg = cg + (sm.y * sm.w) * T;
            cb = cb + (sm.z * sm.w) * T;
            T = T * (1.0f - sm.w);
            return T == 0.0f || T < P.ert_eps;
        };
        constexpr bool kDefer = VR_DEFER_SHADE && SHADE && GF;
        struct Pend {
            FieldRowsT<kHalfField<VT>> g;
            float4 sm;
            float ax, ay, az;
            bool on;
        } X;
        X.on = false;
        auto finish = [&]() -> bool {
            if (!kDefer || !X.on) return false;
            X.on = false;
            float gx, gy_, gz;
            field_rows_filter(X.g, X.ax, X.ay, X.az, gx, gy_, gz);
            phong(P, gx, gy_, gz, d0, d1, d2, X.sm);
            return composite(X.sm);
        };
        auto consume_cell = [&](const Stage &S, const Cell8<VT> &c) -> bool {
            if (kDefer && finish()) return true;
            const float d = c.tri(S.ax, S.ay, S.az);
            const float tt = div_by_range(d - P.vmin, P);
            float4 sm = tf_lookup(s_tf, P.tf_n, P.tf_nf, tt);
            if (!S.slab) sm.w = 0.0f;
            if constexpr (kDefer) {
                if (sm.w > 0.0f) {
                    field_rows_load(reinterpret_cast<const char *>(P.grad), S.ce, X.g);
                    X.sm = sm;
                    X.ax = S.ax;
                    X.ay = S.ay;
                    X.az = S.az;
                    X.on = true;
                }
                return false;
            }
            if (SHADE && sm.w > 0.0f)
                shade_sample<VT, GF, true>(P, vol, S.ce, c, S.pi, S.pj, S.pk, by_stride,
                                           bz_stride, S.ax, S.ay, S.az, d0, d1, d2, sm);
            return composite(sm);
        };
        auto consume = [&](const Stage &S) -> bool {
            Cell8<VT> c;
            c.decode(S.w);
            return consume_cell(S, c);
        };
        auto advance = [&]() {
            p0 = p0 + d0 * P.step;
            p1 = p1 + d1 * P.step;
            p2 = p2 + d2 * P.step;
        };
        Stage A, B;
        int k = 0;
        {
            prep(A, k);
            while (A.ok) {
                advance();
                prep(B, ++k);
                if (consume(A) || !B.ok) break;
                advance();
                prep(A, ++k);
                if (consume(B)) break;
            }
        }
        finish();
    } else
    for (int it = 0; it < nsteps; ++it) {
        const bool interior = (unsigned)(it - 1) < (unsigned)kin;
        if (!interior &&
            (p0 > 1.0f || p1 > 1.0f || p2 > 1.0f || p0 < 0.0f || p1 < 0.0f || p2 < 0.0f))
            break;
        if (COUNT) ++n_steps;
// ... 917 lines not shown
                            !(std::is_unsigned<SrcT>::value && (unsigned long long)v > (unsigned long long)kIntRangeHi);
            bad |= ok ? 0 : 1;
            iv = ok ? (int)v : 0;
        }
        lo = iv < lo ? iv : lo;
        hi = iv > hi ? iv : hi;
    }
#pragma unroll
    for (int off = 32; off > 0; off >>= 1) {
        const int l2 = __shfl_xor(lo, off, 64), h2 = __shfl_xor(hi, off, 64), b2 = __shfl_xor(bad, off, 64);
        lo = l2 < lo ? l2 : lo;
        hi = h2 > hi ? h2 : hi;
        bad |= b2;
    }
    __shared__ int s_lo[4], s_hi[4], s_bad[4];
    const uint32_t w = threadIdx.x >> 6;
    if ((threadIdx.x & 63) == 0) {
        s_lo[w] = lo;
        s_hi[w] = hi;
        s_bad[w] = bad;
    }
    __syncthreads();
    if (threadIdx.x == 0) {
        for (uint32_t i = 1; i < (blockDim.x >> 6); ++i) {
            lo = s_lo[i] < lo ? s_lo[i] : lo;
            hi = s_hi[i] > hi ? s_hi[i] : hi;
            bad |= s_bad[i];
        }
        atomicMin(&out[0], lo);
        atomicMax(&out[1], hi);
        if (bad) atomicOr(&out[2], 1);
    }
}


__device__ __forceinline__ float padded_voxel(const float *__restrict__ bricks, int px, int py,
                                              int pz, uint32_t nx, uint32_t ny, uint32_t nz,
                                              uint32_t nbx, uint32_t nby)
{
    if (px < kPad || py < kPad || pz < kPad || px >= (int)nx + kPad || py >= (int)ny + kPad ||
        pz >= (int)nz + kPad)
        return 0.0f;
    return bricks[kF32VoxelsPerElement * cell_offset<float>(px, py, pz, nbx, nby)];
}

template <typename DstT>
__global__ __launch_bounds__(256) void rebrick_f32_kernel(const float *__restrict__ src,
                                                          float *__restrict__ dst, uint32_t nx,
                                                          uint32_t ny, uint32_t nz, uint32_t snbx,
                                                          uint32_t snby, uint32_t snbz, uint32_t nbx,
                                                          uint32_t nby, size_t nbricks)
{
    using G = GeomOf<DstT>;
    for (size_t bidx = blockIdx.x; bidx < nbricks; bidx += gridDim.x) {
        uint32_t bx, by, bz;
        brick_coords((uint32_t)bidx, nbx, nby, bx, by, bz);
        for (uint32_t l = threadIdx.x; l < (uint32_t)G::Elems; l += blockDim.x) {
            const size_t g = bidx * G::Elems + l;
            const uint32_t lx = l % G::EX, lyz = l / G::EX, lyy = lyz % G::EY, lz = lyz / G::EY;
            const int x = (int)(bx * G::BX + lx) - G::Lo, y = (int)(by * G::BY + lyy) - G::Lo,
                      z = (int)(bz * G::BZ + lz) - G::Lo;
            if constexpr (kPlainF32<DstT>) {
                dst[g] = padded_voxel(src, x, y, z, nx, ny, nz, snbx, snby);
            } else if (kF32VoxelsPerElement == 2 && x >= 0 && y >= 0 && z >= 0 &&
                       x < (int)(snbx * GeomWide::BX) && y < (int)(snby * GeomWide::BY) &&
                       z < (int)(snbz * GeomWide::BZ)) {
                reinterpret_cast<float2 *>(dst)[g] =
                    reinterpret_cast<const float2 *>(src)[cell_offset<float>(x, y, z, snbx, snby)];
            } else {
                reinterpret_cast<float2 *>(dst)[g] =
                    make_float2(padded_voxel(src, x, y, z, nx, ny, nz, snbx, snby),
                                padded_voxel(src, x, y, z + 1, nx, ny, nz, snbx, snby));
            }
        }
    }
}

__global__ __launch_bounds__(256) void rebrick_ymajor_kernel(const float *__restrict__ src,
                                                             float2 *__restrict__ dst, uint32_t nx,
                                                             uint32_t ny, uint32_t nz, uint32_t nbx,
                                                             uint32_t nby, size_t nbricks)
{
    using G = GeomWide;
    for (size_t bidx = blockIdx.x; bidx < nbricks; bidx += gridDim.x) {
        uint32_t bx, by, bz;
        brick_coords((uint32_t)bidx, nbx, nby, bx, by, bz);
        for (uint32_t l = threadIdx.x; l < (uint32_t)G::Elems; l += blockDim.x) {
            const uint32_t lx = l % G::EX, lzy = l / G::EX, lz = lzy % G::EZ, ly = lzy / G::EZ;
            float2 v = make_float2(0.0f, 0.0f);
            if (ly < (uint32_t)G::EY) {
                const int x = (int)(bx * G::BX + lx), y = (int)(by * G::BY + ly),
                          z = (int)(bz * G::BZ + lz);
                v = make_float2(padded_voxel(src, x, y, z, nx, ny, nz, nbx, nby),
                                padded_voxel(src, x, y + 1, z, nx, ny, nz, nbx, nby));
            }
            dst[bidx * G::Elems + l] = v;
        }
    }
}

__device__ __forceinline__ _Float16 field_half(float d, float scale)
{
    float x = d * scale;
    x = x > 65504.0f ? 65504.0f : (x < -65504.0f ? -65504.0f : x);
    return (_Float16)x;
}

template <bool H>
__global__ __launch_bounds__(256) void grad_field_kernel(const float *__restrict__ bricks,
                                                         float *__restrict__ grad, uint32_t nx,
                                                         uint32_t ny, uint32_t nz, uint32_t nbx,
                                                         uint32_t nby, size_t nbricks, float scale)
{
    using G = GeomWide;
    constexpr int LX = G::EX + 2, LY = G::EY + 2 + (H ? 1 : 0), LZ = G::EZ + 3;
    __shared__ float box[LX * LY * LZ];
    __shared__ uint2 ostage[3 * G::Elems];
    uint2 *__restrict__ out = reinterpret_cast<uint2 *>(grad);
    const uint32_t nbz = (uint32_t)(nbricks / ((size_t)nbx * nby));
    for (size_t bidx = blockIdx.x; bidx < nbricks; bidx += gridDim.x) {
        uint32_t bx, by, bz;
        brick_coords((uint32_t)bidx, nbx, nby, bx, by, bz);
        const int x0 = (int)(bx * G::BX) - 1, y0 = (int)(by * G::BY) - 1, z0 = (int)(bz * G::BZ) - 1;
        __syncthreads();
        static_assert(LZ % 2 == 0, "the box is loaded in z-pairs");
        for (int i = (int)threadIdx.x; i < LX * LY * (LZ / 2); i += (int)blockDim.x) {
            const int ix = i % LX, iyz = i / LX, iy = iyz % LY, iz = 2 * (iyz / LY);
            const int px = x0 + ix, py = y0 + iy, pz = z0 + iz;
            float2 v;
            if (kF32VoxelsPerElement == 2 && px >= 0 && py >= 0 && pz >= 0 &&
                px < (int)(nbx * G::BX) && py < (int)(nby * G::BY) && pz < (int)(nbz * G::BZ))
                v = reinterpret_cast<const float2 *>(bricks)[cell_offset<float>(px, py, pz, nbx, nby)];
            else
                v = make_float2(padded_voxel(bricks, px, py, pz, nx, ny, nz, nbx, nby),
                                padded_voxel(bricks, px, py, pz + 1, nx, ny, nz, nbx, nby));
            box[(iz * LY + iy) * LX + ix] = v.x;
            box[((iz + 1) * LY + iy) * LX + ix] = v.y;
        }
        __syncthreads();
        for (uint32_t l = threadIdx.x; l < (uint32_t)G::Elems; l += blockDim.x) {
            const uint32_t lx = l % G::EX, lyz = l / G::EX, lyy = lyz % G::EY, lz = lyz / G::EY;
            uint2 *o = ostage + 3 * l;
            if (lz >= (uint32_t)G::EZ) {
                o[0] = o[1] = o[2] = make_uint2(0u, 0u);
                continue;
            }
            const int c = ((int)lz + 1) * (LX * LY) + ((int)lyy + 1) * LX + ((int)lx + 1);
            if constexpr (H) {
                _Float16 hv[12];
#pragma unroll
                for (int q = 0; q < 4; ++q) {
                    const int cq = c + (q >> 1) * LX + (q & 1) * (LX * LY);
                    auto V = [&](int dx, int dy, int dz) { return box[cq + dx + dy * LX + dz * (LX * LY)]; };
                    hv[0 + q] = field_half(V(1, 0, 0) - V(-1, 0, 0), scale);
                    hv[4 + q] = field_half(V(0, 1, 0) - V(0, -1, 0), scale);
                    hv[8 + q] = field_half(V(0, 0, 1) - V(0, 0, -1), scale);
                }
#pragma unroll
                for (int i = 0; i < 3; ++i) {
                    const h2v lo = {hv[4 * i], hv[4 * i + 1]}, hi = {hv[4 * i + 2], hv[4 * i + 3]};
                    o[i] = make_uint2(__builtin_bit_cast(uint32_t, lo), __builtin_bit_cast(uint32_t, hi));
                }
            } else {
                float d[6];
#pragma unroll
                for (int h = 0; h < 2; ++h) {
                    const int ch = c + h * (LX * LY);
                    auto V = [&](int dx, int dy, int dz) { return box[ch + dx + dy * LX + dz * (LX * LY)]; };
                    d[0 + h] = V(1, 0, 0) - V(-1, 0, 0);
                    d[2 + h] = V(0, 1, 0) - V(0, -1, 0);
                    d[4 + h] = V(0, 0, 1) - V(0, 0, -1);
                }
#pragma unroll
                for (int i = 0; i < 3; ++i)
                    o[i] = make_uint2(__float_as_uint(d[2 * i]), __float_as_uint(d[2 * i + 1]));
            }
        }
        __syncthreads();
        uint2 *__restrict__ ob = out + bidx * (3 * (size_t)G::Elems);
        for (uint32_t j = threadIdx.x; j < 3u * (uint32_t)G::Elems; j += blockDim.x) ob[j] = ostage[j];
    }
}


template <typename VT>
__global__ __launch_bounds__(256) void brick_range_kernel(const VT *__restrict__ bricks,
                                                          uint32_t nbricks, uint32_t per_brick,
                                                          uint32_t nbx, uint32_t nby,
                                                          float2 *__restrict__ range)
{
    const uint32_t lane = threadIdx.x & 63;
    const uint32_t b = blockIdx.x * 4 + (threadIdx.x >> 6);
    if (b >= nbricks) return;
    const VT *src = bricks + (size_t)b * per_brick;
    float lo = INFINITY, hi = -INFINITY;
    bool nan = false;
    for (uint32_t e = lane; e < per_brick; e += 64) {
        const float v = (float)src[e];
        nan = nan || v != v;
        lo = fminf(lo, v);
        hi = fmaxf(hi, v);
    }
#pragma unroll
    for (int off = 32; off > 0; off >>= 1) {
        lo = fminf(lo, __shfl_xor(lo, off, 64));
        hi = fmaxf(hi, __shfl_xor(hi, off, 64));
    }
    const bool any_nan = __ballot(nan) != 0;
    uint32_t bx, by, bz;
    brick_coords(b, nbx, nby, bx, by, bz);
    if (lane == 0) range[(bz * nby + by) * nbx + bx] = any_nan ? make_float2(NAN, NAN) : make_float2(lo, hi);
}

__global__ __launch_bounds__(256) void range_max_kernel(float2 *__restrict__ range, uint32_t nbricks)
{
    __shared__ float s_lo[4], s_hi[4];
    float lo = INFINITY, hi = -INFINITY;
    for (uint32_t b = threadIdx.x; b < nbricks; b += 256) {
        const float2 r = range[b];
        lo = fminf(lo, r.x);
        hi = fmaxf(hi, r.y);
    }
#pragma unroll
    for (int off = 32; off > 0; off >>= 1) {
        lo = fminf(lo, __shfl_xor(lo, off, 64));
        hi = fmaxf(hi, __shfl_xor(hi, off, 64));
    }
    if ((threadIdx.x & 63) == 0) {
        s_lo[threadIdx.x >> 6] = lo;
// ... 294 lines not shown
        case 10: return brick_from<double>(src, dst, nx, ny, nz, storage, s);
        default: return hipErrorInvalidValue;
    }
}

hipError_t launch_generate(int kind, int storage, void *dst, uint32_t nx, uint32_t ny,
                           uint32_t nz, const float *params_dev, int nparams, hipStream_t s)
{
    (void)nparams;
    if (kind != 0) return hipErrorInvalidValue;
    const size_t total = (size_t)nx * ny * nz;
    switch (storage) {
        case ST_U8: hipLaunchKernelGGL((generate_kernel<uint8_t>), dim3(grid_for(total)), dim3(256), 0, s, (uint8_t *)dst, nx, ny, total, params_dev); break;
        case ST_U16: hipLaunchKernelGGL((generate_kernel<uint16_t>), dim3(grid_for(total)), dim3(256), 0, s, (uint16_t *)dst, nx, ny, total, params_dev); break;
        case ST_F32: hipLaunchKernelGGL((generate_kernel<float>), dim3(grid_for(total)), dim3(256), 0, s, (float *)dst, nx, ny, total, params_dev); break;
        default: return hipErrorInvalidValue;
    }
    return hipGetLastError();
}

hipError_t launch_minmax(int storage, const void *linear, size_t count, float *minmax_dev,
                         hipStream_t s)
{
    uint32_t *o = reinterpret_cast<uint32_t *>(minmax_dev);
    const unsigned g = std::min(grid_for(count), 2048u);
    switch (storage) {
        case ST_U8: hipLaunchKernelGGL((minmax_kernel<uint8_t>), dim3(g), dim3(256), 0, s, (const uint8_t *)linear, count, o); break;
        case ST_I8: hipLaunchKernelGGL((minmax_kernel<int8_t>), dim3(g), dim3(256), 0, s, (const int8_t *)linear, count, o); break;
        case ST_U16: hipLaunchKernelGGL((minmax_kernel<uint16_t>), dim3(g), dim3(256), 0, s, (const uint16_t *)linear, count, o); break;
        case ST_I16: hipLaunchKernelGGL((minmax_kernel<int16_t>), dim3(g), dim3(256), 0, s, (const int16_t *)linear, count, o); break;
        default: hipLaunchKernelGGL((minmax_kernel<float>), dim3(g), dim3(256), 0, s, (const float *)linear, count, o); break;
    }
    return hipGetLastError();
}

hipError_t launch_int_range(int src_dtype, const void *src, size_t count, int *out3_dev,
                            hipStream_t s)
{
    const unsigned g = std::min(grid_for(count), 2048u);
    switch (src_dtype) {
        case 5: hipLaunchKernelGGL((int_range_kernel<int32_t>), dim3(g), dim3(256), 0, s, (const int32_t *)src, count, out3_dev); break;
        case 6: hipLaunchKernelGGL((int_range_kernel<uint32_t>), dim3(g), dim3(256), 0, s, (const uint32_t *)src, count, out3_dev); break;
        case 7: hipLaunchKernelGGL((int_range_kernel<int64_t>), dim3(g), dim3(256), 0, s, (const int64_t *)src, count, out3_dev); break;
        case 8: hipLaunchKernelGGL((int_range_kernel<uint64_t>), dim3(g), dim3(256), 0, s, (const uint64_t *)src, count, out3_dev); break;
        case 9: hipLaunchKernelGGL((int_range_kernel<float>), dim3(g), dim3(256), 0, s, (const float *)src, count, out3_dev); break;
        default: return hipErrorInvalidValue;
    }
    return hipGetLastError();
}

hipError_t launch_assemble(const void *gathered, void *out, int out_format, uint32_t W,
                           uint32_t H, uint32_t row_block, uint32_t nranks,
                           uint32_t shard_rows, RowShare share, hipStream_t s)
{
    const unsigned g = grid_for((size_t)W * H);
    if (out_format == 0)
        hipLaunchKernelGGL((assemble_kernel<uint32_t>), dim3(g), dim3(256), 0, s,
                           (const uint32_t *)gathered, (uint32_t *)out, W, H, row_block, nranks,
                           shard_rows, share);
    else
        hipLaunchKernelGGL((assemble_kernel<float4>), dim3(g), dim3(256), 0, s,
                           (const float4 *)gathered, (float4 *)out, W, H, row_block, nranks,
                           shard_rows, share);
    return hipGetLastError();
}

hipError_t launch_brick_range(int storage, const void *bricks, uint32_t nbx, uint32_t nby,
                              uint32_t nbz, float2 *range_dev, hipStream_t s)
{
    const uint32_t nbricks = nbx * nby * nbz;
    const unsigned g = (nbricks + 3) / 4;
    const uint32_t per = (uint32_t)(brick_elems(storage) * voxels_per_element(storage));
    switch (storage & 0xF) {
        case ST_U8: hipLaunchKernelGGL((brick_range_kernel<uint8_t>), dim3(g), dim3(256), 0, s, (const uint8_t *)bricks, nbricks, per, nbx, nby, range_dev); break;
        case ST_I8: hipLaunchKernelGGL((brick_range_kernel<int8_t>), dim3(g), dim3(256), 0, s, (const int8_t *)bricks, nbricks, per, nbx, nby, range_dev); break;
        case ST_U16: hipLaunchKernelGGL((brick_range_kernel<uint16_t>), dim3(g), dim3(256), 0, s, (const uint16_t *)bricks, nbricks, per, nbx, nby, range_dev); break;
        case ST_I16: hipLaunchKernelGGL((brick_range_kernel<int16_t>), dim3(g), dim3(256), 0, s, (const int16_t *)bricks, nbricks, per, nbx, nby, range_dev); break;
        default: hipLaunchKernelGGL((brick_range_kernel<float>), dim3(g), dim3(256), 0, s, (const float *)bricks, nbricks, per, nbx, nby, range_dev); break;
    }
    return hipGetLastError();
}

hipError_t launch_grad_field(const float *bricks, float *grad, uint32_t nx, uint32_t ny,
                             uint32_t nz, bool half, int scale_log2, hipStream_t s)
{
    const uint32_t nbx = bricks_for(nx, 0, ST_F32), nby = bricks_for(ny, 1, ST_F32),
                   nbz = bricks_for(nz, 2, ST_F32);
    const size_t total = (size_t)nbx * nby * nbz;
    const float scale = std::ldexp(1.0f, scale_log2);
    if (half)
        hipLaunchKernelGGL(grad_field_kernel<true>, dim3(grid_bricks(total)), dim3(256), 0, s,
                           bricks, grad, nx, ny, nz, nbx, nby, total, scale);
    else
        hipLaunchKernelGGL(grad_field_kernel<false>, dim3(grid_bricks(total)), dim3(256), 0, s,
                           bricks, grad, nx, ny, nz, nbx, nby, total, scale);
    return hipGetLastError();
}

hipError_t launch_rebrick_f32(const float *src_bricks, void *dst, uint32_t nx, uint32_t ny,
                              uint32_t nz, int storage, hipStream_t s)
{
    const uint32_t snbx = bricks_for(nx, 0, ST_F32), snby = bricks_for(ny, 1, ST_F32),
                   snbz = bricks_for(nz, 2, ST_F32);
    const uint32_t nbx = bricks_for(nx, 0, storage), nby = bricks_for(ny, 1, storage),
                   nbz = bricks_for(nz, 2, storage);
    const size_t total = (size_t)nbx * nby * nbz;
    float *d = static_cast<float *>(dst);
    switch (storage) {
        case ST_F32 | kAltFlag: hipLaunchKernelGGL((rebrick_f32_kernel<F32Alt>), dim3(grid_bricks(total)), dim3(256), 0, s, src_bricks, d, nx, ny, nz, snbx, snby, snbz, nbx, nby, total); break;
        case ST_F32 | kPlainF32Flag: hipLaunchKernelGGL((rebrick_f32_kernel<F32P>), dim3(grid_bricks(total)), dim3(256), 0, s, src_bricks, d, nx, ny, nz, snbx, snby, snbz, nbx, nby, total); break;
        case ST_F32 | kStencilF32Flag: hipLaunchKernelGGL((rebrick_f32_kernel<F32S>), dim3(grid_bricks(total)), dim3(256), 0, s, src_bricks, d, nx, ny, nz, snbx, snby, snbz, nbx, nby, total); break;
        case ST_F32 | kYMajorFlag: hipLaunchKernelGGL(rebrick_ymajor_kernel, dim3(grid_bricks(total)), dim3(256), 0, s, src_bricks, reinterpret_cast<float2 *>(d), nx, ny, nz, snbx, snby, total); break;
        default: return hipErrorInvalidValue;
    }
    return hipGetLastError();
}

hipError_t launch_skip_dist(const float2 *range_dev, uint32_t nbx, uint32_t nby, uint32_t nbz,
                            const uint32_t *tf_nz_dev, int tf_n, float vmin, float vrange,
                            uint8_t *dist_dev, uint8_t *scratch_dev, hipStream_t s)
{
    const uint32_t nb = nbx * nby * nbz;
    const unsigned g = (nb + 255) / 256;
    hipLaunchKernelGGL(classify_kernel, dim3(g), dim3(256), 0, s, range_dev, nb, tf_nz_dev, tf_n,
                       (float)tf_n, vmin, vrange, dist_dev);
    hipLaunchKernelGGL(dist_pass_kernel, dim3(g), dim3(256), 0, s, (const uint8_t *)dist_dev,
                       scratch_dev, nbx, nby, nbz, 0);
    hipLaunchKernelGGL(dist_pass_kernel, dim3(g), dim3(256), 0, s, (const uint8_t *)scratch_dev,
                       dist_dev, nbx, nby, nbz, 1);
    hipLaunchKernelGGL(dist_pass_kernel, dim3(g), dim3(256), 0, s, (const uint8_t *)dist_dev,
                       scratch_dev, nbx, nby, nbz, 2);
    return hipMemcpyAsync(dist_dev, scratch_dev, nb, hipMemcpyDeviceToDevice, s);
}

#ifdef VR_WG_TIMES
hipError_t debug_wg_times_reset()
{
    const unsigned int z = 0;
    return hipMemcpyToSymbol(HIP_SYMBOL(g_wg_count), &z, sizeof(z));
}
hipError_t debug_wg_times_read(unsigned long long *out, unsigned int max, unsigned int *count)
{
    unsigned int n = 0;
    hipError_t e = hipMemcpyFromSymbol(&n, HIP_SYMBOL(g_wg_count), sizeof(n));
    if (e != hipSuccess) return e;
    n = n < kWgTimesMax ? n : kWgTimesMax;
    n = n < max ? n : max;
    *count = n;
    return n ? hipMemcpyFromSymbol(out, HIP_SYMBOL(g_wg_times), 4 * n * sizeof(unsigned long long))
             : hipSuccess;
}
#endif

hipError_t launch_order_tiles(const uint32_t *cost, const uint32_t *lists, uint32_t *perm,
                              uint32_t per_xcd, hipStream_t s)
{
    hipLaunchKernelGGL(order_tiles_kernel, dim3(8), dim3(256), 0, s, cost, lists, perm, per_xcd);
    return hipGetLastError();
}

}
```

volumetric-renderer_amd/vr_amd.py:

```python
from __future__ import annotations

import contextlib
import ctypes as C
import os
from dataclasses import dataclass
from typing import Optional, Sequence

import numpy as np

HERE = os.path.dirname(os.path.abspath(__file__))
LIB_PATH = os.environ.get("VR_AMD_LIB") or os.path.join(HERE, "lib", "libvr_amd.so")

DTYPE_I8, DTYPE_U8, DTYPE_I16, DTYPE_U16, DTYPE_I32, DTYPE_U32 = 1, 2, 3, 4, 5, 6
DTYPE_I64, DTYPE_U64, DTYPE_F32, DTYPE_F64 = 7, 8, 9, 10
NP_TO_DTYPE = {
    np.dtype(np.int8): DTYPE_I8, np.dtype(np.uint8): DTYPE_U8,
    np.dtype(np.int16): DTYPE_I16, np.dtype(np.uint16): DTYPE_U16,
    np.dtype(np.int32): DTYPE_I32, np.dtype(np.uint32): DTYPE_U32,
    np.dtype(np.int64): DTYPE_I64, np.dtype(np.uint64): DTYPE_U64,
    np.dtype(np.float32): DTYPE_F32, np.dtype(np.float64): DTYPE_F64,
}
DTYPE_TO_NP = {v: k for k, v in NP_TO_DTYPE.items()}
STORAGE_BYTES = {0: 1, 1: 1, 2: 2, 3: 2, 4: 4}

OUT_RGBA8, OUT_RGBA32F = 0, 1


class vr_camera(C.Structure):
    _fields_ = [("view", C.c_float * 16), ("position", C.c_float * 3),
                ("fovy_deg", C.c_float), ("znear", C.c_float), ("zfar", C.c_float)]


class vr_params(C.Structure):
    _fields_ = [("step", C.c_float), ("ray_dist", C.c_float), ("ert_eps", C.c_float),
                ("shading", C.c_int32), ("clear_color", C.c_float * 4),
                ("ambient", C.c_float), ("diffuse", C.c_float), ("specular", C.c_float),
                ("spec_power", C.c_int32), ("tile_order", C.c_int32),
                ("skip_empty", C.c_int32), ("wave_shape", C.c_int32),
                ("frames_in_flight", C.c_int32), ("exact_gradient", C.c_int32),
                ("depth_zero_to_one", C.c_int32)]


class vr_stats(C.Structure):
    _fields_ = [("rays", C.c_uint64), ("samples", C.c_uint64),
                ("shaded_samples", C.c_uint64), ("steps", C.c_uint64),
                ("skipped_samples", C.c_uint64)]


class vr_orbit_camera(C.Structure):
    _fields_ = [("center", C.c_float * 3), ("orientation", C.c_float * 4),
                ("radius", C.c_float)]


class vr_memory_info(C.Structure):
    _fields_ = [(n, C.c_uint64) for n in (
        "volume_bytes", "field_bytes", "oblique_copy_bytes", "plain_copy_bytes",
        "stencil_copy_bytes", "skip_bytes", "derived_bytes", "budget_bytes",
        "builds", "evictions", "downgrades", "last_downgrade")]


class vr_dist_host_profile(C.Structure):
    _fields_ = [("frames", C.c_uint64)] + [(n, C.c_double) for n in (
        "render_us", "gather_us", "assemble_us", "record_us", "wait_us", "total_us")]


DERIVED = {1: "field", 2: "oblique_copy", 3: "plain_copy", 4: "stencil_copy", 5: "skip",
           6: "ymajor_copy"}


class vr_member_timing(C.Structure):
    _fields_ = [("device", C.c_int32), ("frames", C.c_uint64), ("kernel_ms", C.c_double),
                ("render_ms", C.c_double), ("gather_ms", C.c_double), ("assemble_ms", C.c_double)]


class vr_variant_facts(C.Structure):
    _fields_ = [(n, C.c_int32) for n in (
        "layout", "mode", "shade", "count", "skip", "field", "field_half", "pipeline", "tf_n",
        "pair", "mip_inflight")]


class vr_mpr_plane(C.Structure):
    _fields_ = [("origin", C.c_float * 3), ("du", C.c_float * 3), ("dv", C.c_float * 3),
                ("dn", C.c_float * 3), ("width", C.c_uint32), ("height", C.c_uint32),
                ("nsamples", C.c_uint32), ("op", C.c_int32)]


class vr_dataset(C.Structure):
    _fields_ = [("dims", C.c_uint32 * 3), ("dtype", C.c_int), ("data", C.c_void_p),
                ("vmin", C.c_float), ("vmax", C.c_float)]


ABI_SYMBOLS = [
    "vr_abi_version", "vr_params_default", "vr_create", "vr_destroy", "vr_last_error",
    "vr_create_mask", "vr_get_device_mask",
    "vr_resize", "vr_get_size", "vr_get_device", "vr_set_volume", "vr_set_volume_device", "vr_generate_volume",
    "vr_volume_bytes", "vr_debug_read_volume", "vr_debug_read_volume_native", "vr_debug_volume_info",
    "vr_set_transfer_function", "vr_set_slicing", "vr_render", "vr_render_device",
    "vr_shard_rows", "vr_assemble_rows", "vr_count_work", "vr_timing_enable",
    "vr_timing_read", "vr_timing_reset", "vr_kernel_name",
    "vr_import_memory_fd", "vr_release_external_memory",
    "vr_set_row_share", "vr_get_row_share", "vr_shard_rows_ctx",
    "vr_set_memory_budget", "vr_memory_report", "vr_prepare",
]
HOST_SYMBOLS = [
    "vr_cam_init", "vr_cam_rotate", "vr_cam_zoom", "vr_cam_position", "vr_cam_view",
    "vr_cam_to_camera", "vr_gradient_create", "vr_gradient_destroy",
    "vr_gradient_add_color_marker", "vr_gradient_add_alpha_marker",
    "vr_gradient_remove_color_marker", "vr_gradient_remove_alpha_marker",
    "vr_gradient_set_alpha_marker", "vr_gradient_set_color_marker", "vr_gradient_marker_count",
    "vr_gradient_sample", "vr_gradient_discretize", "vr_nrrd_load", "vr_nrrd_write_raw",
    "vr_csv_load", "vr_dataset_free", "vr_host_last_error",
]

DIST_SYMBOLS = [
    "vr_dist_unique_id", "vr_dist_create", "vr_dist_render", "vr_dist_synchronize",
    "vr_dist_last_error", "vr_dist_destroy", "vr_dist_timing_enable", "vr_dist_timing_read",
    "vr_dist_host_profile_enable", "vr_dist_host_profile_read",
]
DIST_ID_BYTES = 128
DEBUG_SYMBOLS = ["vr_debug_set_knob", "vr_debug_get_knob", "vr_debug_timing_member",
                 "vr_debug_create_members", "vr_debug_fail_member",
                 "vr_debug_host_profile_enable", "vr_debug_host_profile_member",
                 "vr_debug_variant_name", "vr_debug_last_kernel_name",
                 "vr_debug_ymajor_copy_bytes"]
MODES_SYMBOLS = ["vr_set_render_mode", "vr_get_render_mode"]
MODE_COMPOSITE, MODE_MIP = 0, 1
MODE_ISO = 3
MODE_MINIP, MODE_MEAN = 4, 6
ISO_SYMBOLS = ["vr_set_isovalue", "vr_get_isovalue"]
MPR_SYMBOLS = ["vr_mpr_render", "vr_mpr_render_device", "vr_mpr_count_work", "vr_mpr_axis_plane"]
OP_MAX, OP_MIN, OP_MEAN = 0, 1, 2
MPR_MAX_SAMPLES = 4096
AXIS_SAGITTAL, AXIS_CORONAL, AXIS_AXIAL = 0, 1, 2
EXCHANGE_RCCL, EXCHANGE_COPY = 0, 1
KNOBS = {"pipeline": 1, "pair": 2, "pair_lanes": 3, "grad_field": 4, "u8_layout": 6,
         "tile_order": 7, "narrow": 8, "alt_geometry": 9, "mip_inflight": 10}
KNOB_AUTO = {"pipeline": -1, "pair": -1, "pair_lanes": 0, "grad_field": -1,
             "u8_layout": -1, "tile_order": 0, "narrow": 1, "alt_geometry": -1,
             "mip_inflight": 0}

ABI_VERSION = 9
_LIB = None


def lib() -> C.CDLL:
    global _LIB
    if _LIB is not None:
        return _LIB
    if not os.path.exists(LIB_PATH):
        raise RuntimeError(f"{LIB_PATH} is missing: build it with `make -C volumetric-renderer_amd` "
                           "(or __graft_entry__.build()); there is no CPU fallback")
    try:
        import torch
    except ImportError:
        pass
    L = C.CDLL(LIB_PATH)
    vp, u32, f32, i32 = C.c_void_p, C.c_uint32, C.c_float, C.c_int
    sig = {
        "vr_abi_version": (i32, []),
        "vr_params_default": (None, [C.POINTER(vr_params)]),
        "vr_create": (vp, [i32, u32, u32]),
        "vr_destroy": (None, [vp]),
        "vr_last_error": (C.c_char_p, [vp]),
        "vr_resize": (i32, [vp, u32, u32]),
        "vr_get_size": (i32, [vp, C.POINTER(u32), C.POINTER(u32)]),
        "vr_get_device": (i32, [vp, C.POINTER(i32)]),
        "vr_create_mask": (vp, [u32, u32, u32]),
        "vr_get_device_mask": (i32, [vp, C.POINTER(u32)]),
        "vr_dist_unique_id": (i32, [vp]),
        "vr_dist_create": (vp, [vp, vp, i32, i32, u32, i32]),
        "vr_dist_render": (i32, [vp, C.POINTER(vr_camera), C.POINTER(vr_params), vp, vp]),
        "vr_dist_synchronize": (i32, [vp]),
        "vr_dist_last_error": (C.c_char_p, [vp]),
        "vr_dist_destroy": (None, [vp]),
        "vr_dist_timing_enable": (i32, [vp, i32]),
        "vr_dist_host_profile_enable": (i32, [vp, i32]),
        "vr_dist_host_profile_read": (i32, [vp, C.POINTER(vr_dist_host_profile)]),
        "vr_dist_timing_read": (i32, [vp, C.POINTER(C.c_double), C.POINTER(C.c_double),
                                      C.POINTER(C.c_uint64)]),
        "vr_set_volume": (i32, [vp, vp, i32, u32, u32, u32, f32, f32]),
        "vr_set_volume_device": (i32, [vp, vp, i32, u32, u32, u32, f32, f32, vp]),
        "vr_generate_volume": (i32, [vp, i32, i32, u32, u32, u32, u32, C.POINTER(f32), C.POINTER(f32)]),
        "vr_volume_bytes": (C.c_uint64, [vp]),
        "vr_debug_read_volume": (i32, [vp, vp]),
        "vr_debug_read_volume_native": (i32, [vp, vp]),
        "vr_debug_volume_info": (i32, [vp, C.POINTER(u32), C.POINTER(f32), C.POINTER(i32)]),
        "vr_set_transfer_function": (i32, [vp, C.POINTER(u32), u32]),
        "vr_set_slicing": (i32, [vp, C.POINTER(f32), C.POINTER(f32)]),
        "vr_render": (i32, [vp, C.POINTER(vr_camera), C.POINTER(vr_params), vp, i32]),
        "vr_render_device": (i32, [vp, C.POINTER(vr_camera), C.POINTER(vr_params), vp, i32, u32, u32, u32, vp]),
        "vr_shard_rows": (u32, [u32, u32, u32]),
        "vr_assemble_rows": (i32, [vp, vp, vp, i32, u32, u32, vp]),
        "vr_count_work": (i32, [vp, C.POINTER(vr_camera), C.POINTER(vr_params), u32, u32, u32, C.POINTER(vr_stats)]),
        "vr_timing_enable": (i32, [vp, i32]),
        "vr_timing_read": (i32, [vp, C.POINTER(C.c_double), C.POINTER(C.c_uint64)]),
        "vr_timing_reset": (i32, [vp]),
        "vr_kernel_name": (C.c_char_p, [vp, C.POINTER(vr_params)]),
        "vr_import_memory_fd": (C.c_int, [vp, C.c_int, C.c_uint64, C.c_uint64, C.POINTER(vp),
                                          C.POINTER(vp)]),
        "vr_release_external_memory": (C.c_int, [vp, vp]),
        "vr_debug_set_knob": (i32, [vp, i32, i32]),
        "vr_debug_timing_member": (i32, [vp, i32, C.POINTER(vr_member_timing)]),
        "vr_debug_host_profile_enable": (i32, [vp, i32]),
        "vr_debug_host_profile_member": (i32, [vp, i32, C.POINTER(vr_dist_host_profile)]),
        "vr_set_row_share": (i32, [vp, u32, u32]),
        "vr_get_row_share": (i32, [vp, C.POINTER(u32), C.POINTER(u32)]),
        "vr_shard_rows_ctx": (u32, [vp, u32, u32, u32]),
        "vr_set_memory_budget": (i32, [vp, C.c_uint64]),
        "vr_memory_report": (i32, [vp, C.POINTER(vr_memory_info)]),
        "vr_prepare": (i32, [vp, C.POINTER(vr_camera), C.POINTER(vr_params)]),
        "vr_debug_get_knob": (i32, [vp, i32, C.POINTER(i32)]),
        "vr_set_render_mode": (i32, [vp, i32]),
        "vr_get_render_mode": (i32, [vp, C.POINTER(i32)]),
        "vr_set_isovalue": (i32, [vp, C.c_float]),
        "vr_get_isovalue": (i32, [vp, C.POINTER(C.c_float)]),
        "vr_mpr_render": (i32, [vp, C.POINTER(vr_mpr_plane), C.POINTER(vr_params), vp, i32]),
        "vr_mpr_render_device": (i32, [vp, C.POINTER(vr_mpr_plane), C.POINTER(vr_params), vp, i32, vp]),
        "vr_mpr_count_work": (i32, [vp, C.POINTER(vr_mpr_plane), C.POINTER(vr_params),
                                    C.POINTER(vr_stats)]),
        "vr_mpr_axis_plane": (i32, [i32, f32, u32, u32, u32, f32, i32, C.POINTER(vr_mpr_plane)]),
        "vr_debug_create_members": (vp, [C.POINTER(i32), i32, u32, u32, i32]),
        "vr_debug_fail_member": (i32, [vp, i32, C.c_uint64]),
        "vr_debug_variant_name": (i32, [C.POINTER(vr_variant_facts), C.c_char_p, C.c_size_t]),
        "vr_debug_last_kernel_name": (C.c_char_p, [vp]),
        "vr_debug_ymajor_copy_bytes": (C.c_uint64, [vp]),
        "vr_cam_init": (None, [C.POINTER(vr_orbit_camera)]),
        "vr_cam_rotate": (None, [C.POINTER(vr_orbit_camera), f32, f32]),
        "vr_cam_zoom": (None, [C.POINTER(vr_orbit_camera), f32]),
        "vr_cam_position": (None, [C.POINTER(vr_orbit_camera), C.POINTER(f32)]),
        "vr_cam_view": (None, [C.POINTER(vr_orbit_camera), C.POINTER(f32)]),
        "vr_cam_to_camera": (None, [C.POINTER(vr_orbit_camera), C.POINTER(vr_camera)]),
        "vr_gradient_create": (vp, []),
        "vr_gradient_destroy": (None, [vp]),
        "vr_gradient_add_color_marker": (i32, [vp, f32, f32, f32, f32]),
        "vr_gradient_add_alpha_marker": (i32, [vp, f32, f32]),
        "vr_gradient_remove_color_marker": (i32, [vp, C.c_size_t]),
        "vr_gradient_remove_alpha_marker": (i32, [vp, C.c_size_t]),
        "vr_gradient_set_alpha_marker": (i32, [vp, C.c_size_t, f32, f32]),
        "vr_gradient_set_color_marker": (i32, [vp, C.c_size_t, f32, f32, f32, f32]),
        "vr_gradient_marker_count": (C.c_size_t, [vp, i32]),
        "vr_gradient_sample": (None, [vp, f32, C.POINTER(f32)]),
        "vr_gradient_discretize": (i32, [vp, C.c_size_t, C.POINTER(u32)]),
        "vr_nrrd_load": (i32, [C.c_char_p, C.POINTER(vr_dataset)]),
        "vr_nrrd_write_raw": (i32, [C.c_char_p, vp, i32, C.POINTER(u32)]),
        "vr_csv_load": (i32, [C.POINTER(C.c_char_p), C.c_size_t, C.POINTER(vr_dataset)]),
        "vr_dataset_free": (None, [C.POINTER(vr_dataset)]),
        "vr_host_last_error": (C.c_char_p, []),
    }
    for name, (res, args) in sig.items():
        fn = getattr(L, name)
        fn.restype = res
        fn.argtypes = args
    if L.vr_abi_version() != ABI_VERSION:
        raise RuntimeError(f"{LIB_PATH} has ABI {L.vr_abi_version()}, this binding expects "
                           f"{ABI_VERSION}: rebuild it")
    _LIB = L
    return L


def mpr_plane(origin, du, dv, dn, width: int, height: int, nsamples: int = 1,
              op: int = OP_MAX) -> vr_mpr_plane:
    pl = vr_mpr_plane()
    for name, v in (("origin", origin), ("du", du), ("dv", dv), ("dn", dn)):
        for a in range(3):
            getattr(pl, name)[a] = float(v[a])
    pl.width, pl.height, pl.nsamples, pl.op = int(width), int(height), int(nsamples), int(op)
    return pl


def axis_plane(axis: int, position: float, width: int, height: int, nsamples: int = 1,
               spacing: float = 0.0, op: int = OP_MAX) -> vr_mpr_plane:
    pl = vr_mpr_plane()
    rc = lib().vr_mpr_axis_plane(int(axis), float(position), int(width), int(height), int(nsamples),
                                 float(spacing), int(op), C.byref(pl))
    if rc != 0:
        raise ValueError(f"vr_mpr_axis_plane failed ({rc}): {lib().vr_last_error(None).decode()}")
    return pl


def default_params(**overrides) -> vr_params:
    p = vr_params()
    lib().vr_params_default(C.byref(p))
    for k, v in overrides.items():
        if k == "clear_color":
            for i in range(4):
                p.clear_color[i] = v[i]
        else:
            setattr(p, k, v)
    return p


class OrbitCamera:

    def __init__(self):
        self._c = vr_orbit_camera()
        lib().vr_cam_init(C.byref(self._c))

    def rotate(self, dx: float, dy: float) -> "OrbitCamera":
        lib().vr_cam_rotate(C.byref(self._c), dx, dy)
        return self

    def zoom(self, delta: float) -> "OrbitCamera":
        lib().vr_cam_zoom(C.byref(self._c), delta)
        return self

    def set_radius(self, r: float) -> "OrbitCamera":
        self._c.radius = r
        return self
# ... 261 lines not shown

    def render_mpr_device(self, plane: vr_mpr_plane, params: Optional[vr_params], out_ptr: int,
                          out_format: int = OUT_RGBA8, stream: int = 0):
        p = params if params is not None else default_params()
        self._check(lib().vr_mpr_render_device(self._ctx, C.byref(plane), C.byref(p),
                                               C.c_void_p(out_ptr), out_format,
                                               C.c_void_p(stream or None)), "render_mpr_device")

    def count_work_mpr(self, plane: vr_mpr_plane, params: Optional[vr_params] = None) -> dict:
        p = params if params is not None else default_params()
        st = vr_stats()
        self._check(lib().vr_mpr_count_work(self._ctx, C.byref(plane), C.byref(p), C.byref(st)),
                    "count_work_mpr")
        return dict(rays=st.rays, samples=st.samples, shaded_samples=st.shaded_samples,
                    steps=st.steps, skipped_samples=st.skipped_samples)

    def render_device(self, camera, params, out_ptr: int, out_format: int = OUT_RGBA8,
                      row_block: int = 16, rank: int = 0, nranks: int = 1, stream: int = 0):
        cam = camera.to_vr_camera() if isinstance(camera, OrbitCamera) else camera
        self._check(lib().vr_render_device(self._ctx, C.byref(cam), C.byref(params),
                                           C.c_void_p(out_ptr), out_format, row_block, rank,
                                           nranks, C.c_void_p(stream or None)), "render_device")

    def assemble_rows(self, gathered_ptr: int, out_ptr: int, out_format: int, row_block: int,
                      nranks: int, stream: int = 0):
        self._check(lib().vr_assemble_rows(self._ctx, C.c_void_p(gathered_ptr), C.c_void_p(out_ptr),
                                           out_format, row_block, nranks, C.c_void_p(stream or None)),
                    "assemble_rows")

    def count_work(self, camera, params, row_block=16, rank=0, nranks=1) -> dict:
        cam = camera.to_vr_camera() if isinstance(camera, OrbitCamera) else camera
        st = vr_stats()
        self._check(lib().vr_count_work(self._ctx, C.byref(cam), C.byref(params), row_block, rank,
                                        nranks, C.byref(st)), "count_work")
        return dict(rays=st.rays, samples=st.samples, shaded_samples=st.shaded_samples,
                    steps=st.steps, skipped_samples=st.skipped_samples)

    def timing_enable(self, on: bool = True):
        self._check(lib().vr_timing_enable(self._ctx, 1 if on else 0), "timing_enable")

    def timing_read(self):
        ms, n = C.c_double(), C.c_uint64()
        self._check(lib().vr_timing_read(self._ctx, C.byref(ms), C.byref(n)), "timing_read")
        return float(ms.value), int(n.value)

    def timing_reset(self):
        self._check(lib().vr_timing_reset(self._ctx), "timing_reset")

    def kernel_name(self, params) -> str:
        return lib().vr_kernel_name(self._ctx, C.byref(params)).decode()

    def last_kernel_name(self) -> str:
        return lib().vr_debug_last_kernel_name(self._ctx).decode()

    def timing_member(self, member: int) -> dict:
        t = vr_member_timing()
        self._check(lib().vr_debug_timing_member(self._ctx, member, C.byref(t)), "timing_member")
        return dict(device=int(t.device), frames=int(t.frames), kernel_ms=float(t.kernel_ms),
                    render_ms=float(t.render_ms), gather_ms=float(t.gather_ms),
                    assemble_ms=float(t.assemble_ms))

    def fail_member(self, member: int, frame: int):
        self._check(lib().vr_debug_fail_member(self._ctx, member, frame), "vr_debug_fail_member")

    def set_row_share(self, first_weight: int, other_weight: int):
        self._check(lib().vr_set_row_share(self._ctx, first_weight, other_weight), "set_row_share")

    def row_share(self):
        a, b = C.c_uint32(), C.c_uint32()
        self._check(lib().vr_get_row_share(self._ctx, C.byref(a), C.byref(b)), "row_share")
        return int(a.value), int(b.value)

    def shard_rows(self, height: int, row_block: int, nranks: int) -> int:
        return int(lib().vr_shard_rows_ctx(self._ctx, height, row_block, nranks))

    def set_memory_budget(self, nbytes: int):
        self._check(lib().vr_set_memory_budget(self._ctx, C.c_uint64(nbytes)), "set_memory_budget")

    def memory_report(self) -> dict:
        m = vr_memory_info()
        self._check(lib().vr_memory_report(self._ctx, C.byref(m)), "memory_report")
        r = {n: int(getattr(m, n)) for n, _ in vr_memory_info._fields_}
        r["ymajor_copy_bytes"] = int(lib().vr_debug_ymajor_copy_bytes(self._ctx))
        return r

    def prepare(self, camera, params):
        cam = camera.to_vr_camera() if isinstance(camera, OrbitCamera) else camera
        self._check(lib().vr_prepare(self._ctx, C.byref(cam), C.byref(params)), "prepare")

    def host_profile_enable(self, on: bool = True):
        self._check(lib().vr_debug_host_profile_enable(self._ctx, int(bool(on))), "host_profile_enable")

    def host_profile_member(self, member: int) -> dict:
        h = vr_dist_host_profile()
        self._check(lib().vr_debug_host_profile_member(self._ctx, member, C.byref(h)),
                    "host_profile_member")
        n = max(int(h.frames), 1)
        return dict(frames=int(h.frames), **{k: getattr(h, k) / n for k, _ in vr_dist_host_profile._fields_[1:]})

    def set_knob(self, name: str, value: int):
        self._check(lib().vr_debug_set_knob(self._ctx, KNOBS[name], int(value)), f"set_knob({name})")

    def get_knob(self, name: str) -> int:
        v = C.c_int()
        self._check(lib().vr_debug_get_knob(self._ctx, KNOBS[name], C.byref(v)), f"get_knob({name})")
        return int(v.value)

    @contextlib.contextmanager
    def knobs(self, **kw):
        for k, v in kw.items():
            self.set_knob(k, v)
        try:
            yield self
        finally:
            for k in kw:
                self.set_knob(k, KNOB_AUTO[k])


def dist_unique_id() -> bytes:
    buf = C.create_string_buffer(DIST_ID_BYTES)
    rc = lib().vr_dist_unique_id(buf)
    if rc:
        raise RuntimeError(f"vr_dist_unique_id failed ({rc}): {lib().vr_dist_last_error(None).decode()}")
    return buf.raw


class DistFrames:

    def __init__(self, rp: "OffscreenPass", uid: bytes, nranks: int, rank: int,
                 row_block: int = 8, frames_in_flight: int = 3):
        if len(uid) != DIST_ID_BYTES:
            raise ValueError("communicator id must be DIST_ID_BYTES bytes")
        self.rank, self.nranks = rank, nranks
        self._rp = rp
        self._d = lib().vr_dist_create(rp._ctx, C.create_string_buffer(uid, DIST_ID_BYTES),
                                       nranks, rank, row_block, frames_in_flight)
        if not self._d:
            raise RuntimeError(f"vr_dist_create failed: {lib().vr_dist_last_error(None).decode()}")

    def _check(self, rc: int, what: str):
        if rc:
            raise RuntimeError(f"{what} failed ({rc}): {lib().vr_dist_last_error(self._d).decode()}")

    def render(self, camera, params, frame_ptr: int = 0, stream: int = 0):
        cam = camera.to_vr_camera() if isinstance(camera, OrbitCamera) else camera
        self._check(lib().vr_dist_render(self._d, C.byref(cam), C.byref(params),
                                         C.c_void_p(frame_ptr or None), C.c_void_p(stream or None)),
                    "vr_dist_render")

    def synchronize(self):
        self._check(lib().vr_dist_synchronize(self._d), "vr_dist_synchronize")

    def timing_enable(self, on: bool = True):
        self._check(lib().vr_dist_timing_enable(self._d, 1 if on else 0), "vr_dist_timing_enable")

    def host_profile(self, enable=None):
        if enable is not None:
            self._check(lib().vr_dist_host_profile_enable(self._d, 1 if enable else 0),
                        "vr_dist_host_profile_enable")
            return None
        h = vr_dist_host_profile()
        self._check(lib().vr_dist_host_profile_read(self._d, C.byref(h)), "vr_dist_host_profile_read")
        n = max(int(h.frames), 1)
        return dict(frames=int(h.frames), **{k: getattr(h, k) / n for k, _ in vr_dist_host_profile._fields_[1:]})

    def timing_read(self):
# ... 97 lines not shown
```

Measured before the change: 393.8.

## Add y-major ordered half-precision gradient field alongside the y-major volume copy

```diff
diff --git a/include/vr/vr.h b/include/vr/vr.h
--- a/include/vr/vr.h
+++ b/include/vr/vr.h
@@ -138,7 +138,8 @@
     VR_DERIVED_PLAIN_COPY = 3,
     VR_DERIVED_STENCIL_COPY = 4,
     VR_DERIVED_SKIP = 5,
-    VR_DERIVED_YMAJOR_COPY = 6
+    VR_DERIVED_YMAJOR_COPY = 6,
+    VR_DERIVED_YMAJOR_FIELD = 7
 };
 #define VR_MEMORY_BUDGET_UNLIMITED (~(uint64_t)0)
 #define VR_MEMORY_BUDGET_DEFAULT (~(uint64_t)0 - 1)
diff --git a/include/vr/vr_debug.h b/include/vr/vr_debug.h
--- a/include/vr/vr_debug.h
+++ b/include/vr/vr_debug.h
@@ -17,7 +17,8 @@
     VR_KNOB_TILE_ORDER = 7,
     VR_KNOB_NARROW = 8,
     VR_KNOB_ALT_GEOMETRY = 9,
-    VR_KNOB_MIP_INFLIGHT = 10
+    VR_KNOB_MIP_INFLIGHT = 10,
+    VR_KNOB_FIELD_ORDER = 11
 };
 
 typedef struct vr_member_timing {
@@ -47,6 +48,7 @@
 const char *vr_debug_last_kernel_name(const vr_ctx *ctx);
 
 uint64_t vr_debug_ymajor_copy_bytes(const vr_ctx *ctx);
+uint64_t vr_debug_ymajor_field_bytes(const vr_ctx *ctx);
 
 #ifdef __cplusplus
 }
diff --git a/volumetric-renderer_amd/csrc/vr_api.hip b/volumetric-renderer_amd/csrc/vr_api.hip
--- a/volumetric-renderer_amd/csrc/vr_api.hip
+++ b/volumetric-renderer_amd/csrc/vr_api.hip
@@ -60,6 +60,10 @@
     bool grad_valid = false;
     uint64_t grad_used = 0;
     bool grad_half = false;
+    float *ygrad = nullptr;
+    size_t ygrad_bytes = 0;
+    bool ygrad_valid = false;
+    int ygrad_scale_log2 = 0;
     int grad_scale_log2 = 0;
     float data_lo = 0.0f, data_hi = 1.0f;
     struct TileSched {
@@ -104,7 +108,7 @@
     uint64_t timed_launches = 0;
     struct Knobs {
         int pipeline = -1, pair = -1, pair_lanes = 0, grad_field = -1, u8_layout = -1,
-            tile_order = 0, narrow = 1, alt = -1, mip_inflight = 0;
+            tile_order = 0, narrow = 1, alt = -1, mip_inflight = 0, field_order = -1;
     } knobs;
     std::vector<vr_ctx *> members;
     vr::Group *group = nullptr;
@@ -356,7 +360,7 @@
 int set_bricks(vr_ctx *c, int storage, uint32_t nx, uint32_t ny, uint32_t nz, void **out)
 {
     c->range_valid = c->dist_valid = false;
-    c->grad_valid = false;
+    c->grad_valid = c->ygrad_valid = false;
     for (auto &a : c->alt) a.valid = a.failed = false;
     const size_t bytes = (size_t)bricks_for(nx, 0, storage) * bricks_for(ny, 1, storage) *
                          bricks_for(nz, 2, storage) * brick_elems(storage) * element_size(storage);
@@ -565,6 +569,7 @@
     P.nz = c->nz;
     P.nbx = bricks_for(c->nx, 0, c->layout);
     P.nby = bricks_for(c->ny, 1, c->layout);
+    P.nbz = bricks_for(c->nz, 2, c->layout);
     P.fnx = (float)c->nx;
     P.fny = (float)c->ny;
     P.fnz = (float)c->nz;
@@ -635,7 +640,7 @@
 constexpr size_t kSkipBytesPerBrick = sizeof(float2) + 2;
 size_t derived_bytes(const vr_ctx *c)
 {
-    size_t b = c->grad ? c->grad_bytes : 0;
+    size_t b = (c->grad ? c->grad_bytes : 0) + (c->ygrad ? c->ygrad_bytes : 0);
     for (const auto &a : c->alt)
         if (a.bricks) b += a.bytes + kBrickSlackBytes;
     return b + c->nbricks_alloc * kSkipBytesPerBrick;
@@ -711,7 +716,7 @@
 }
 constexpr int kYMajorAlt = 3;
 int make_room(vr_ctx *c, size_t extra, size_t replaced, int keep_alt, bool keep_field, hipStream_t s,
-              bool *fits)
+              bool *fits, bool keep_yfield = false)
 {
     *fits = budget_allows(c, extra, replaced);
     while (!*fits) {
@@ -727,8 +732,14 @@
                 oldest = c->alt[i].used;
             }
         if (keep_alt != kYMajorAlt && c->alt[kYMajorAlt].bricks) pick = kYMajorAlt;
+        if (c->ygrad && !keep_yfield) pick = -3;
         if (pick == -2) return VR_OK;
-        if (pick == -1) {
+        if (pick == -3) {
+            if (int rc = release_async(c, c->ygrad, s)) return rc;
+            c->ygrad = nullptr;
+            c->ygrad_bytes = 0;
+            c->ygrad_valid = false;
+        } else if (pick == -1) {
             if (int rc = release_async(c, c->grad, s)) return rc;
             c->grad = nullptr;
             c->grad_bytes = 0;
@@ -748,6 +759,10 @@
     c->grad = nullptr;
     c->grad_bytes = 0;
     c->grad_valid = false;
+    if (c->ygrad) (void)hipFreeAsync(c->ygrad, nullptr);
+    c->ygrad = nullptr;
+    c->ygrad_bytes = 0;
+    c->ygrad_valid = false;
     for (auto &a : c->alt) {
         if (a.bricks) (void)hipFreeAsync(a.bricks, nullptr);
         a = vr_ctx::AltCopy();
@@ -866,7 +881,7 @@
     }
     if (!c->grad_valid) {
         if (launch_grad_field(static_cast<const float *>(c->bricks), c->grad, c->nx, c->ny, c->nz,
-                              half, k, s) != hipSuccess)
+                              half, k, false, s) != hipSuccess)
             return built;
         built = true;
         ++c->n_builds;
@@ -902,7 +917,8 @@
         if (!P.skip_empty) *refused = VR_DERIVED_SKIP;
     }
     bool g_refused = false;
-    const bool g_built = p->shading && ensure_grad(c, P, s, p->exact_gradient == 0, &g_refused);
+    const bool g_built = p->shading && !P.grad_ymajor &&
+                         ensure_grad(c, P, s, p->exact_gradient == 0, &g_refused);
     if (g_refused) *refused = VR_DERIVED_FIELD;
     const bool built = (!r0 && c->range_valid) || (!d0 && c->dist_valid) || g_built;
     if (built) return record_build(c, s);
@@ -970,12 +986,13 @@
 {
     const vr_ctx::Knobs &k = c->knobs;
     return k.pipeline < 0 && k.pair < 0 && k.pair_lanes == 0 && k.grad_field < 0 && k.alt < 0 &&
-           k.tile_order == 0;
+           k.tile_order == 0 && k.field_order < 0;
 }
 bool want_ymajor(const vr_ctx *c, const vr_params *p, bool field, bool field_half, bool pipelined)
 {
     if (!pipelined || c->tf_n > (uint32_t)kTfLds) return false;
-    if (p->shading ? !(field && field_half && p->exact_gradient == 0) : field) return false;
+    if (c->brick_bytes / element_size(ST_F32) >= 0xFFFF0000ull) return false;
+    if (p->shading ?!(field && field_half && p->exact_gradient == 0) : field) return false;
     if (c->knobs.alt >= 0) return c->knobs.alt == 5;
     return knobs_default(c) && c->dense_rows && c->ray_axis == 1 &&
            c->brick_bytes > kInfinityCacheBytes;
@@ -1066,6 +1083,62 @@
     return record_build(c, s);
 }
 
+#ifndef VR_YFIELD_POLICY
+#define VR_YFIELD_POLICY 1
+#endif
+bool yfield_wanted(const vr_ctx *c, const vr_params *p, bool pipelined)
+{
+    if (c->layout != ST_F32 || !p->shading || p->skip_empty || p->exact_gradient != 0) return false;
+    if (c->knobs.field_order == 0 || !use_grad_field(c, true)) return false;
+    if (!want_ymajor(c, p, true, true, pipelined)) return false;
+    return c->knobs.field_order == 1 || (VR_YFIELD_POLICY && c->knobs.alt < 0);
+}
+int ensure_yfield(vr_ctx *c, MarchParams &P, hipStream_t s, bool *got)
+{
+    *got = false;
+    bool ready = false;
+    if (int rc = ensure_alt(c, ST_F32 | kYMajorFlag, s, &ready)) return rc;
+    if (!ready) return VR_OK;
+    const int k = field_scale_log2(c->data_lo, c->data_hi);
+    const size_t bytes = c->brick_bytes / element_size(ST_F32) * kGradElemBytes;
+    if (c->ygrad && c->ygrad_bytes != bytes) {
+        if (int rc = release_async(c, c->ygrad, s)) return rc;
+        c->ygrad = nullptr;
+        c->ygrad_bytes = 0;
+        c->ygrad_valid = false;
+    }
+    if (!c->ygrad) {
+        if (!budget_allows(c, bytes, 0)) return VR_OK;
+        size_t free_b = 0, total_b = 0;
+        void *g = nullptr;
+        if (hipMemGetInfo(&free_b, &total_b) != hipSuccess || free_b < bytes + (2ull << 30) ||
+            hipMallocAsync(&g, bytes, s) != hipSuccess) {
+            (void)hipGetLastError();
+            return VR_OK;
+        }
+        c->ygrad = static_cast<float *>(g);
+        c->ygrad_bytes = bytes;
+        c->ygrad_valid = false;
+    }
+    if (!c->ygrad_valid || c->ygrad_scale_log2 != k) {
+        if (c->ygrad_valid)
+            if (int rc = fence_others(c, s)) return rc;
+        c->ygrad_valid = false;
+        const hipError_t e = launch_grad_field(static_cast<const float *>(c->bricks), c->ygrad,
+                                               c->nx, c->ny, c->nz, true, k, true, s);
+        if (e != hipSuccess) return hip_fail(c, e, "y-major difference field");
+        c->ygrad_valid = true;
+        c->ygrad_scale_log2 = k;
+        ++c->n_builds;
+        if (int rc = record_build(c, s)) return rc;
+    }
+    P.grad = c->ygrad;
+    P.grad_half = 1;
+    P.grad_ymajor = 1;
+    *got = true;
+    return VR_OK;
+}
+
 VariantFacts launch_facts(const vr_ctx *c, const vr_params *p, const MarchParams &P, int layout,
                           bool count)
 {
@@ -1087,10 +1160,13 @@
         return f;
     }
     f.skip = p && p->skip_empty;
-    f.field = f.shade && use_grad_field(c, p->exact_gradient == 0) && c->grad && c->grad_valid;
-    f.field_half = f.field && p->exact_gradient == 0;
     const uint32_t tiles = ((c->width + 15) / 16) * ((c->height + kMarchRows - 1) / kMarchRows);
     f.pipeline = use_pipeline(f.shade, tiles, c);
+    const bool yfield = f.shade && yfield_wanted(c, p, f.pipeline != 0) && c->ygrad &&
+                        c->ygrad_valid && c->alt[kYMajorAlt].valid;
+    f.field = f.shade && use_grad_field(c, p->exact_gradient == 0) &&
+              ((c->grad && c->grad_valid) || yfield);
+    f.field_half = f.field && p->exact_gradient == 0;
     if (p)
         if (const int lay = want_alt(c, p, false, f.field != 0, f.field_half != 0, f.pipeline != 0);
             lay != c->layout && c->alt[alt_index(lay)].valid)
@@ -1206,7 +1282,7 @@
             d->vmax = src->vmax;
             d->data_lo = src->data_lo;
             d->data_hi = src->data_hi;
-            d->range_valid = d->dist_valid = d->grad_valid = false;
+            d->range_valid = d->dist_valid = d->grad_valid = d->ygrad_valid = false;
         }
     }
     for (size_t k = 1; k < n; ++k)
@@ -1238,6 +1314,7 @@
         case VR_KNOB_NARROW: return &c->knobs.narrow;
         case VR_KNOB_ALT_GEOMETRY: return &c->knobs.alt;
         case VR_KNOB_MIP_INFLIGHT: return &c->knobs.mip_inflight;
+        case VR_KNOB_FIELD_ORDER: return &c->knobs.field_order;
         default: return nullptr;
     }
 }
@@ -2003,6 +2080,12 @@
         rc = ensure_mip(c, p, P, M, s, &refused);
         if (rc) return rc;
     } else {
+        if (yfield_wanted(c, p, P.pipelined != 0) && !use_pair(c, P, p)) {
+            bool got = false;
+            if ((rc = wait_builds(c, s)) != VR_OK || (rc = ensure_yfield(c, P, s, &got)) != VR_OK)
+                return rc;
+            if (!got && c->knobs.field_order == 1) refused = VR_DERIVED_YMAJOR_FIELD;
+        }
         rc = ensure_derived(c, p, P, s, &refused);
         if (rc) return rc;
         if (use_pair(c, P, p)) {
@@ -2024,11 +2107,14 @@
                 P.vol_bytes = c->alt[alt_index(lay)].bytes;
                 P.nbx = bricks_for(c->nx, 0, layout);
                 P.nby = bricks_for(c->ny, 1, layout);
+                P.nbz = bricks_for(c->nz, 2, layout);
             } else {
                 if (!(lay & kYMajorFlag) || c->knobs.alt == 5) refused = alt_derived_code(lay);
             }
         }
     }
+    if (P.grad_ymajor && !(layout & kYMajorFlag))
+        return fail(c, VR_EIO, "internal: the y-major field without the y-major copy");
     if (!launch) return VR_OK;
     if (refused) {
         ++c->n_downgrades;
@@ -2245,8 +2331,12 @@
     uint32_t refused = 0;
     MipArgs M{nullptr, 0};
     const bool mip = range_mode(c);
+    const bool no_field = !mip && !(c->grad && c->grad_valid) &&
+                          yfield_wanted(c, p, P.pipelined != 0) && !use_pair(c, P, p);
+    if (no_field) P.grad_ymajor = 1;
     rc = mip ? ensure_mip(c, p, P, M, nullptr, &refused) : ensure_derived(c, p, P, nullptr, &refused);
     if (rc) return rc;
+    P.grad_ymajor = 0;
     HIP_TRY(c, hipMemset(c->counters, 0, 8 * sizeof(unsigned long long)), "hipMemset(counters)");
     FrameVariant v;
     resolve_variant(launch_facts(c, p, P, c->layout, true), &v);
@@ -2413,6 +2503,13 @@
     thread_local std::string name;
     name = c->last_mpr_name.empty() ? variant_kernel_name(c->last_variant) : c->last_mpr_name;
     return name.c_str();
+}
+
+uint64_t vr_debug_ymajor_field_bytes(const vr_ctx *c)
+{
+    if (!c) return 0;
+    if (is_group(c)) return vr_debug_ymajor_field_bytes(c->members[0]);
+    return c->ygrad ? c->ygrad_bytes : 0;
 }
 
 uint64_t vr_debug_ymajor_copy_bytes(const vr_ctx *c)
diff --git a/volumetric-renderer_amd/csrc/vr_internal.h b/volumetric-renderer_amd/csrc/vr_internal.h
--- a/volumetric-renderer_amd/csrc/vr_internal.h
+++ b/volumetric-renderer_amd/csrc/vr_internal.h
@@ -140,27 +140,46 @@
 {
     return GeomWide::EX * (GeomWide::BY * (int)zl - GeomWide::BZ * (int)yl);
 }
+__host__ __device__ constexpr uint32_t ymajor_slot(uint32_t bx, uint32_t by, uint32_t bz,
+                                                   uint32_t nbx, uint32_t nbz)
+{
+    return bx + nbx * (bz + nbz * by);
+}
+__host__ __device__ constexpr void ymajor_coords(uint32_t slot, uint32_t nbx, uint32_t nbz,
+                                                 uint32_t &bx, uint32_t &by, uint32_t &bz)
+{
+    bx = slot % nbx;
+    bz = (slot / nbx) % nbz;
+    by = slot / (nbx * nbz);
+}
 __host__ __device__ constexpr size_t ymajor_cell_offset(uint32_t pi, uint32_t pj, uint32_t pk,
-                                                        uint32_t nbx, uint32_t nby,
+                                                        uint32_t nbx, uint32_t nbz,
                                                         int *field_delta = nullptr)
 {
     using G = GeomWide;
     const uint32_t bx = pi / G::BX, by = pj / G::BY, bz = pk / G::BZ;
     const uint32_t xl = pi - bx * G::BX, yl = pj - by * G::BY, zl = pk - bz * G::BZ;
     if (field_delta) *field_delta = ymajor_field_delta(yl, zl);
-    return (size_t)brick_slot(bx, by, bz, nbx, nby) * (size_t)G::Elems + ymajor_local(xl, yl, zl);
+    return (size_t)ymajor_slot(bx, by, bz, nbx, nbz) * (size_t)G::Elems + ymajor_local(xl, yl, zl);
 }
 namespace ymajor_check {
+template <uint32_t NBX, uint32_t NBY, uint32_t NBZ>
 constexpr bool map_ok()
 {
     using G = GeomWide;
-    constexpr uint32_t nbx = (3 + kGroupMask) & ~kGroupMask, nby = (2 + kGroupMask) & ~kGroupMask,
-                       nbz = nby;
+    constexpr uint32_t nbx = NBX, nby = NBY, nbz = NBZ;
+    bool slot_seen[nbx * nby * nbz] = {};
     for (uint32_t bz = 0; bz < nbz; ++bz)
         for (uint32_t by = 0; by < nby; ++by)
             for (uint32_t bx = 0; bx < nbx; ++bx) {
+                const uint32_t slot = ymajor_slot(bx, by, bz, nbx, nbz);
+                if (slot >= nbx * nby * nbz || slot_seen[slot]) return false;
+                slot_seen[slot] = true;
+                uint32_t cx = 0, cy = 0, cz = 0;
+                ymajor_coords(slot, nbx, nbz, cx, cy, cz);
+                if (cx != bx || cy != by || cz != bz) return false;
                 bool seen[G::EX * G::EY * G::EZ] = {};
-                const size_t base = (size_t)brick_slot(bx, by, bz, nbx, nby) * (size_t)G::Elems;
+                const size_t base = (size_t)slot * (size_t)G::Elems;
                 for (uint32_t zl = 0; zl < (uint32_t)G::EZ; ++zl)
                     for (uint32_t yl = 0; yl < (uint32_t)G::EY; ++yl)
                         for (uint32_t xl = 0; xl < (uint32_t)G::EX; ++xl) {
@@ -172,14 +191,15 @@
                             if (xl < (uint32_t)G::BX && yl < (uint32_t)G::BY && zl < (uint32_t)G::BZ) {
                                 int fd = 0;
                                 const size_t e = ymajor_cell_offset(bx * G::BX + xl, by * G::BY + yl,
-                                                                    bz * G::BZ + zl, nbx, nby, &fd);
+                                                                    bz * G::BZ + zl, nbx, nbz, &fd);
                                 if (e != base + l || fd != ymajor_field_delta(yl, zl)) return false;
                             }
                         }
             }
     return true;
 }
-static_assert(map_ok(), "the y-major map is a bijection onto each brick, 72 (zl - yl) from z-major");
+static_assert(map_ok<3, 2, 2>(), "the y-major maps are bijections, 72 (zl - yl) from z-major");
+static_assert(map_ok<2, 1, 3>() && map_ok<1, 3, 2>(), "... also where nby != nbz");
 static_assert(GeomWide::BX != 8 || GeomWide::BY != 8 || GeomWide::BZ != 8 ||
                   ymajor_field_delta(3, 5) == 72 * (5 - 3),
               "8^3 cells: l_zmajor - l_ymajor == 72 (zl - yl)");
@@ -316,6 +336,8 @@
     float inv_range;
     uint32_t share_w0, share_w;
     unsigned long long vol_bytes, out_bytes;
+    uint32_t nbz;
+    int32_t grad_ymajor;
 };
 
 struct MipArgs {
@@ -407,7 +429,8 @@
 constexpr int kSkipCap = 16;
 constexpr size_t kGradElemBytes = 24;
 hipError_t launch_grad_field(const float *bricks, float *grad, uint32_t nx, uint32_t ny,
-                             uint32_t nz, bool half, int scale_log2, hipStream_t stream);
+                             uint32_t nz, bool half, int scale_log2, bool ymajor,
+                             hipStream_t stream);
 hipError_t launch_rebrick_f32(const float *src_bricks, void *dst, uint32_t nx, uint32_t ny,
                               uint32_t nz, int storage, hipStream_t stream);
 inline int field_scale_log2(float vmin, float vmax)
diff --git a/volumetric-renderer_amd/csrc/vr_kernels.hip b/volumetric-renderer_amd/csrc/vr_kernels.hip
--- a/volumetric-renderer_amd/csrc/vr_kernels.hip
+++ b/volumetric-renderer_amd/csrc/vr_kernels.hip
@@ -1056,7 +1056,7 @@
     if constexpr (PIPE) {
         struct Stage {
             CellRaw<VT> w;
-            size_t ce;
+            std::conditional_t<kYMajor<VT>, uint32_t, size_t> ce;
             float ax, ay, az;
             int pi, pj, pk;
             bool ok, slab;
@@ -1077,11 +1077,11 @@
             S.pj = j + kPad;
             S.pk = kk + kPad;
             if constexpr (kYMajor<VT>) {
-                S.ce = cell_offset<float>(S.pi, S.pj, S.pk, P.nbx, P.nby);
-                size_t e = (size_t)((long)S.ce -
-                                    ymajor_field_delta((uint32_t)S.pj % (uint32_t)G::BY,
-                                                       (uint32_t)S.pk % (uint32_t)G::BZ));
-                if (VR_OOB(3, e * kElemBytes<VT>, P.vol_bytes)) e = S.ce = 0;
+                uint32_t e = (uint32_t)cell_offset<VT>(S.pi, S.pj, S.pk, P.nbx, P.nbz);
+                S.ce = (!SHADE || P.grad_ymajor)
+                           ? e
+                           : (uint32_t)cell_offset<float>(S.pi, S.pj, S.pk, P.nbx, P.nby);
+                if (VR_OOB(3, (size_t)e * kElemBytes<VT>, P.vol_bytes)) e = S.ce = 0;
                 Cell8<VT>::issue(S.w, vol, e);
             } else {
                 S.ce = cell_offset<VT>(S.pi, S.pj, S.pk, P.nbx, P.nby);
@@ -2165,9 +2165,10 @@
                                                              uint32_t nby, size_t nbricks)
 {
     using G = GeomWide;
+    const uint32_t nbz = (uint32_t)(nbricks / ((size_t)nbx * nby));
     for (size_t bidx = blockIdx.x; bidx < nbricks; bidx += gridDim.x) {
         uint32_t bx, by, bz;
-        brick_coords((uint32_t)bidx, nbx, nby, bx, by, bz);
+        ymajor_coords((uint32_t)bidx, nbx, nbz, bx, by, bz);
         for (uint32_t l = threadIdx.x; l < (uint32_t)G::Elems; l += blockDim.x) {
             const uint32_t lx = l % G::EX, lzy = l / G::EX, lz = lzy % G::EZ, ly = lzy / G::EZ;
             float2 v = make_float2(0.0f, 0.0f);
@@ -2193,7 +2194,8 @@
 __global__ __launch_bounds__(256) void grad_field_kernel(const float *__restrict__ bricks,
                                                          float *__restrict__ grad, uint32_t nx,
                                                          uint32_t ny, uint32_t nz, uint32_t nbx,
-                                                         uint32_t nby, size_t nbricks, float scale)
+                                                         uint32_t nby, size_t nbricks, float scale,
+                                                         uint32_t ymajor)
 {
     using G = GeomWide;
     constexpr int LX = G::EX + 2, LY = G::EY + 2 + (H ? 1 : 0), LZ = G::EZ + 3;
@@ -2203,7 +2205,10 @@
     const uint32_t nbz = (uint32_t)(nbricks / ((size_t)nbx * nby));
     for (size_t bidx = blockIdx.x; bidx < nbricks; bidx += gridDim.x) {
         uint32_t bx, by, bz;
-        brick_coords((uint32_t)bidx, nbx, nby, bx, by, bz);
+        if (H && ymajor)
+            ymajor_coords((uint32_t)bidx, nbx, nbz, bx, by, bz);
+        else
+            brick_coords((uint32_t)bidx, nbx, nby, bx, by, bz);
         const int x0 = (int)(bx * G::BX) - 1, y0 = (int)(by * G::BY) - 1, z0 = (int)(bz * G::BZ) - 1;
         __syncthreads();
         static_assert(LZ % 2 == 0, "the box is loaded in z-pairs");
@@ -2228,6 +2233,7 @@
                 o[0] = o[1] = o[2] = make_uint2(0u, 0u);
                 continue;
             }
+            if (H && ymajor) o = ostage + 3 * ymajor_local(lx, lyy, lz);
             const int c = ((int)lz + 1) * (LX * LY) + ((int)lyy + 1) * LX + ((int)lx + 1);
             if constexpr (H) {
                 _Float16 hv[12];
@@ -2688,18 +2694,19 @@
 }
 
 hipError_t launch_grad_field(const float *bricks, float *grad, uint32_t nx, uint32_t ny,
-                             uint32_t nz, bool half, int scale_log2, hipStream_t s)
-{
+                             uint32_t nz, bool half, int scale_log2, bool ymajor, hipStream_t s)
+{
+    if (ymajor && !half) return hipErrorInvalidValue;
     const uint32_t nbx = bricks_for(nx, 0, ST_F32), nby = bricks_for(ny, 1, ST_F32),
                    nbz = bricks_for(nz, 2, ST_F32);
     const size_t total = (size_t)nbx * nby * nbz;
     const float scale = std::ldexp(1.0f, scale_log2);
     if (half)
         hipLaunchKernelGGL(grad_field_kernel<true>, dim3(grid_bricks(total)), dim3(256), 0, s,
-                           bricks, grad, nx, ny, nz, nbx, nby, total, scale);
+                           bricks, grad, nx, ny, nz, nbx, nby, total, scale, ymajor ? 1u : 0u);
     else
         hipLaunchKernelGGL(grad_field_kernel<false>, dim3(grid_bricks(total)), dim3(256), 0, s,
-                           bricks, grad, nx, ny, nz, nbx, nby, total, scale);
+                           bricks, grad, nx, ny, nz, nbx, nby, total, scale, 0u);
     return hipGetLastError();
 }
 
diff --git a/volumetric-renderer_amd/vr_amd.py b/volumetric-renderer_amd/vr_amd.py
--- a/volumetric-renderer_amd/vr_amd.py
+++ b/volumetric-renderer_amd/vr_amd.py
@@ -65,7 +65,7 @@
 
 
 DERIVED = {1: "field", 2: "oblique_copy", 3: "plain_copy", 4: "stencil_copy", 5: "skip",
-           6: "ymajor_copy"}
+           6: "ymajor_copy", 7: "ymajor_field"}
 
 
 class vr_member_timing(C.Structure):
@@ -122,7 +122,7 @@
                  "vr_debug_create_members", "vr_debug_fail_member",
                  "vr_debug_host_profile_enable", "vr_debug_host_profile_member",
                  "vr_debug_variant_name", "vr_debug_last_kernel_name",
-                 "vr_debug_ymajor_copy_bytes"]
+                 "vr_debug_ymajor_copy_bytes", "vr_debug_ymajor_field_bytes"]
 MODES_SYMBOLS = ["vr_set_render_mode", "vr_get_render_mode"]
 MODE_COMPOSITE, MODE_MIP = 0, 1
 MODE_ISO = 3
@@ -134,10 +134,10 @@
 AXIS_SAGITTAL, AXIS_CORONAL, AXIS_AXIAL = 0, 1, 2
 EXCHANGE_RCCL, EXCHANGE_COPY = 0, 1
 KNOBS = {"pipeline": 1, "pair": 2, "pair_lanes": 3, "grad_field": 4, "u8_layout": 6,
-         "tile_order": 7, "narrow": 8, "alt_geometry": 9, "mip_inflight": 10}
+         "tile_order": 7, "narrow": 8, "alt_geometry": 9, "mip_inflight": 10, "field_order": 11}
 KNOB_AUTO = {"pipeline": -1, "pair": -1, "pair_lanes": 0, "grad_field": -1,
              "u8_layout": -1, "tile_order": 0, "narrow": 1, "alt_geometry": -1,
-             "mip_inflight": 0}
+             "mip_inflight": 0, "field_order": -1}
 
 ABI_VERSION = 9
 _LIB = None
@@ -224,6 +224,7 @@
         "vr_debug_variant_name": (i32, [C.POINTER(vr_variant_facts), C.c_char_p, C.c_size_t]),
         "vr_debug_last_kernel_name": (C.c_char_p, [vp]),
         "vr_debug_ymajor_copy_bytes": (C.c_uint64, [vp]),
+        "vr_debug_ymajor_field_bytes": (C.c_uint64, [vp]),
         "vr_cam_init": (None, [C.POINTER(vr_orbit_camera)]),
         "vr_cam_rotate": (None, [C.POINTER(vr_orbit_camera), f32, f32]),
         "vr_cam_zoom": (None, [C.POINTER(vr_orbit_camera), f32]),
@@ -651,6 +652,7 @@
         self._check(lib().vr_memory_report(self._ctx, C.byref(m)), "memory_report")
         r = {n: int(getattr(m, n)) for n, _ in vr_memory_info._fields_}
         r["ymajor_copy_bytes"] = int(lib().vr_debug_ymajor_copy_bytes(self._ctx))
+        r["ymajor_field_bytes"] = int(lib().vr_debug_ymajor_field_bytes(self._ctx))
         return r
 
     def prepare(self, camera, params):
```

Result: faster. 401.2 (median of 6 runs) (+1.9%).
